# MinhZou/SNGNN

Hardware: NVIDIA B200
Metric: simknn_build_gpairs_per_s (higher is better)
Workload: dtype f16 tensor-core scores + f32 exact rescore

## Files before the change

### sngnn_b200/csrc/sng_simknn.cu

```cuda
#include "sng_common.cuh"
#include <cuda.h>
#include <cuda_fp16.h>
#include <math_constants.h>
#include <stdlib.h>

namespace sng {
namespace knn {

constexpr int BM = 128;
constexpr int BN = 256;
constexpr int BK = 64;
constexpr int kTileBytes = 128 * BK * 2;
constexpr int kUmmaK = 16;
constexpr int kNonEpiThreads = 128;
constexpr int kMaxStages = 10;
constexpr int kMaxD = 4096;
constexpr int kMaxCandTotal = 192;
constexpr uint32_t kPeerMask = 0xFEFFFFFFu;
#ifdef SNG_KNN_INSTRUMENT
constexpr bool kInstr = true;
#else
constexpr bool kInstr = false;
#endif
#ifdef SNG_KNN_EVTRACE
constexpr bool kEvTrace = true;
#else
constexpr bool kEvTrace = false;
#endif
constexpr int kQueue = 256;
constexpr int kSeedGroups = 16;
constexpr float kQScale = 32512.0f, kQOff = 1.0078125f, kQBin = 1.0f / 32512.0f;
__device__ __forceinline__ unsigned short q_of(float v) {
    const int q = __float2int_rd((v + kQOff) * kQScale);
    return (unsigned short)min(max(q, 0), 65535);
}
__device__ __forceinline__ float q_upper(unsigned q) { return ((float)q + 1.5f) * kQBin - kQOff; }

__device__ __forceinline__ uint32_t smem_u32(const void* p) { return (uint32_t)__cvta_generic_to_shared(p); }
__device__ __forceinline__ uint32_t cluster_ctarank() { uint32_t r; asm volatile("mov.u32 %0, %%cluster_ctarank;" : "=r"(r)); return r; }
__device__ __forceinline__ void cluster_sync_all() {
    asm volatile("barrier.cluster.arrive.release.aligned;" ::: "memory");
    asm volatile("barrier.cluster.wait.acquire.aligned;" ::: "memory");
}
__device__ __forceinline__ bool elect_one() {
    uint32_t p;
    asm volatile("{\n\t.reg .pred p;\n\telect.sync _|p, 0xffffffff;\n\tselp.u32 %0, 1, 0, p;\n\t}" : "=r"(p));
    return p != 0;
}
__device__ __forceinline__ void mbar_init(uint32_t bar, uint32_t count) {
    asm volatile("mbarrier.init.shared::cta.b64 [%0], %1;" ::"r"(bar), "r"(count) : "memory");
}
__device__ __forceinline__ void mbar_expect_tx(uint32_t bar, uint32_t bytes) {
    asm volatile("mbarrier.arrive.expect_tx.shared::cta.b64 _, [%0], %1;" ::"r"(bar), "r"(bytes) : "memory");
}
__device__ __forceinline__ void mbar_arrive_cluster(uint32_t bar, uint32_t cta) {
    asm volatile("{\n\t.reg .b32 ra;\n\tmapa.shared::cluster.u32 ra, %0, %1;\n\tmbarrier.arrive.shared::cluster.b64 _, [ra];\n\t}"
                 ::"r"(bar), "r"(cta) : "memory");
}
__device__ __forceinline__ bool mbar_try(uint32_t bar, uint32_t parity) {
    uint32_t done;
    asm volatile("{\n\t.reg .pred p;\n\tmbarrier.try_wait.parity.shared::cta.b64 p, [%1], %2;\n\tselp.u32 %0, 1, 0, p;\n\t}"
                 : "=r"(done) : "r"(bar), "r"(parity) : "memory");
    return done != 0;
}
__device__ __forceinline__ uint32_t mapa_cluster(uint32_t addr, uint32_t cta) {
    uint32_t ra;
    asm volatile("mapa.shared::cluster.u32 %0, %1, %2;" : "=r"(ra) : "r"(addr), "r"(cta));
    return ra;
}
__device__ __forceinline__ void mbar_arrive_remote(uint32_t cluster_addr) {
    asm volatile("mbarrier.arrive.shared::cluster.b64 _, [%0];" ::"r"(cluster_addr) : "memory");
}
__device__ __noinline__ void mbar_wait_slow(uint32_t bar, uint32_t parity) {
    uint32_t done, polls = 0;
    unsigned long long t0 = 0;
    while (true) {
        asm volatile("{\n\t.reg .pred p;\n\tmbarrier.try_wait.parity.shared::cta.b64 p, [%1], %2;\n\tselp.u32 %0, 1, 0, p;\n\t}"
                     : "=r"(done) : "r"(bar), "r"(parity) : "memory");
        if (done) return;
        if (++polls > 4096u) {
            unsigned long long now;
            asm volatile("mov.u64 %0, %%globaltimer;" : "=l"(now));
            if (t0 == 0) t0 = now;
            else if (now - t0 > 4000000000ull) __trap();
        }
    }
}
__device__ __forceinline__ void mbar_wait(uint32_t bar, uint32_t parity) {
    if (!mbar_try(bar, parity)) mbar_wait_slow(bar, parity);
}
__device__ __forceinline__ void tma_load_2d_pair(uint32_t dst, const CUtensorMap* map, uint32_t bar_leader, int c0, int c1) {
    asm volatile("cp.async.bulk.tensor.2d.cta_group::2.shared::cluster.global.mbarrier::complete_tx::bytes [%0], [%1, {%3, %4}], [%2];"
                 ::"r"(dst), "l"(reinterpret_cast<uint64_t>(map)), "r"(bar_leader), "r"(c0), "r"(c1) : "memory");
}
__device__ __forceinline__ void tc_fence_before() { asm volatile("tcgen05.fence::before_thread_sync;" ::: "memory"); }
__device__ __forceinline__ void tc_fence_after() { asm volatile("tcgen05.fence::after_thread_sync;" ::: "memory"); }
__device__ __forceinline__ void umma_f16_pair(uint32_t tmem_d, uint64_t adesc, uint64_t bdesc, uint32_t idesc, uint32_t accumulate) {
    asm volatile("{\n\t.reg .pred p;\n\tsetp.ne.b32 p, %4, 0;\n\ttcgen05.mma.cta_group::2.kind::f16 [%0], %1, %2, %3, p;\n\t}"
                 ::"r"(tmem_d), "l"(adesc), "l"(bdesc), "r"(idesc), "r"(accumulate) : "memory");
}
__device__ __forceinline__ void umma_commit_pair(uint32_t bar) {
    asm volatile("tcgen05.commit.cta_group::2.mbarrier::arrive::one.shared::cluster.multicast::cluster.b64 [%0], %1;"
                 ::"r"(bar), "h"((uint16_t)3) : "memory");
}
__device__ __forceinline__ void tmem_ld32(uint32_t taddr, uint32_t (&v)[32]) {
    asm volatile(
        "tcgen05.ld.sync.aligned.32x32b.x32.b32 "
        "{%0,%1,%2,%3,%4,%5,%6,%7,%8,%9,%10,%11,%12,%13,%14,%15,%16,%17,%18,%19,%20,%21,%22,%23,%24,%25,%26,%27,%28,%29,%30,%31}, [%32];"
        : "=r"(v[0]), "=r"(v[1]), "=r"(v[2]), "=r"(v[3]), "=r"(v[4]), "=r"(v[5]), "=r"(v[6]), "=r"(v[7]), "=r"(v[8]), "=r"(v[9]),
          "=r"(v[10]), "=r"(v[11]), "=r"(v[12]), "=r"(v[13]), "=r"(v[14]), "=r"(v[15]), "=r"(v[16]), "=r"(v[17]), "=r"(v[18]),
          "=r"(v[19]), "=r"(v[20]), "=r"(v[21]), "=r"(v[22]), "=r"(v[23]), "=r"(v[24]), "=r"(v[25]), "=r"(v[26]), "=r"(v[27]),
          "=r"(v[28]), "=r"(v[29]), "=r"(v[30]), "=r"(v[31])
        : "r"(taddr) : "memory");
}
__device__ __forceinline__ void tmem_ld_wait() { asm volatile("tcgen05.wait::ld.sync.aligned;" ::: "memory"); }
__device__ __forceinline__ float max3(float a, float b, float c) {
    float r;
    asm("max.f32 %0, %1, %2, %3;" : "=f"(r) : "f"(a), "f"(b), "f"(c));
    return r;
}
__device__ __forceinline__ float select32(const uint32_t (&v)[32], int i) {
    uint32_t a[16], b[8], c[4], d[2];
#pragma unroll
    for (int j = 0; j < 16; ++j) a[j] = (i & 1) ? v[2 * j + 1] : v[2 * j];
#pragma unroll
    for (int j = 0; j < 8; ++j) b[j] = (i & 2) ? a[2 * j + 1] : a[2 * j];
#pragma unroll
    for (int j = 0; j < 4; ++j) c[j] = (i & 4) ? b[2 * j + 1] : b[2 * j];
#pragma unroll
    for (int j = 0; j < 2; ++j) d[j] = (i & 8) ? c[2 * j + 1] : c[2 * j];
    return __uint_as_float((i & 16) ? d[1] : d[0]);
}

__device__ __forceinline__ uint64_t make_smem_desc(uint32_t saddr) {
    return (uint64_t)((saddr & 0x3FFFFu) >> 4) | ((uint64_t)(1024u >> 4) << 32) | (1ull << 46) | (2ull << 61);
}
constexpr uint32_t kIdesc = (1u << 4) | ((uint32_t)(BN >> 3) << 17) | ((uint32_t)(256 >> 4) << 24);

struct Stage1Params {
    int nq, n, q_offset;
    int kblocks, ksteps_last;
    int stages;
    int stream_a;
    int cand;
    int qcap;
    int nsplit, tiles_total;
    float thr_lo;
    int remove_self;
    int issuers;
    int debug;
    float* cand_val;
    int* cand_idx;
    float* cand_min;
    const float* seeds;
    float* seed_out;
    int seed_q, seed_stride;
    const int* nq_dev;
    const int* row_ids;
    int* phase;
    long long* trace;
};

template <int W, int NI>
__device__ __forceinline__ void issue_split(const Stage1Params& p, uint32_t base, uint32_t a_off, uint32_t b_off, uint32_t bar_full, uint32_t bar_empty,
                                            uint32_t bar_tfull, uint32_t bar_tempty, int t_beg, int t_end, bool issuer, int lane) {
    constexpr uint32_t kIdescHalf = (1u << 4) | ((uint32_t)(128 >> 3) << 17) | ((uint32_t)(256 >> 4) << 24);
    long long* const trc = kInstr ? p.trace : nullptr;
    const uint64_t adesc0 = make_smem_desc(base + a_off);
    const uint64_t bdesc0 = make_smem_desc(base + b_off);
    const int kb2 = p.kblocks == 2;
    const int ks0 = kb2 ? 4 : p.ksteps_last;
    const int ks1 = kb2 ? p.ksteps_last : 0;
    const int nst = p.stages, step = NI * p.kblocks;
    int st0 = (W * p.kblocks) % nst;
    uint32_t ph0 = (uint32_t)((W * p.kblocks) / nst) & 1u;
    for (int tt = W; tt < t_end - t_beg; tt += NI) {
        const int st1 = st0 + 1;
        const uint32_t acc_phase = (uint32_t)(tt >> 1) & 1u;
        const int acc0 = 2 * (tt & 1);
        const uint64_t b0 = bdesc0 + (uint64_t)(st0 * (kTileBytes >> 4)), b1 = bdesc0 + (uint64_t)(st1 * (kTileBytes >> 4));
        mbar_wait(bar_full + 8 * st0, ph0);
        mbar_wait(bar_tempty + 8 * (tt & 1), acc_phase ^ 1);
        tc_fence_after();
#pragma unroll
        for (int h = 0; h < 2; ++h) {
            if (h == 0 && trc && blockIdx.x == 0 && blockIdx.y == 0 && tt < 64 && lane == 0) trc[tt * 8 + 0] = clock64();
            const uint32_t tmem_d = (uint32_t)((acc0 + h) * 128);
            const uint64_t hb = (uint64_t)(h * (kTileBytes >> 5));
            if (issuer) {
#pragma unroll
                for (int ks = 0; ks < 4; ++ks)
                    if (ks < ks0) umma_f16_pair(tmem_d, adesc0 + (uint64_t)(ks * 2), b0 + hb + (uint64_t)(ks * 2), kIdescHalf, ks != 0 ? 1u : 0u);
#pragma unroll
                for (int ks = 0; ks < 4; ++ks)
                    if (ks < ks1) umma_f16_pair(tmem_d, adesc0 + (uint64_t)((kTileBytes >> 4) + ks * 2), b1 + hb + (uint64_t)(ks * 2), kIdescHalf, 1u);
                if (h == 1) umma_commit_pair(bar_empty + 8 * st0);
                umma_commit_pair(bar_tfull + 8 * (acc0 + h));
            }
            __syncwarp();
        }
        if (trc && blockIdx.x == 0 && blockIdx.y == 0 && tt < 64 && lane == 0) trc[tt * 8 + 1] = clock64();
        st0 += step;
        while (st0 >= nst) { st0 -= nst; ph0 ^= 1u; }
    }
}

template <int EW, bool SEED>
__global__ void __cluster_dims__(2, 1, 1) __launch_bounds__(kNonEpiThreads + 128 * EW, 1)
simknn_stage1_kernel(const __grid_constant__ CUtensorMap map_q, const __grid_constant__ CUtensorMap map_db, const Stage1Params p) {
    constexpr int CPT = BN / EW;
    constexpr bool SPLIT = (EW == 4);
    const int dbg = kInstr ? p.debug : 0;
    long long* const trc = kInstr ? p.trace : nullptr;
    const int nq_eff = p.nq_dev ? min(__ldg(p.nq_dev), p.nq) : p.nq;
    if ((int)(blockIdx.x >> 1) * 2 * BM >= nq_eff) return;
    extern __shared__ uint8_t smem_raw[];
    const uint32_t base = (smem_u32(smem_raw) + 1023u) & ~1023u;
    uint8_t* smem = smem_raw + (base - smem_u32(smem_raw));

    const int warp = threadIdx.x >> 5, lane = threadIdx.x & 31;
    const uint32_t rank = cluster_ctarank();
    const uint32_t a_off = 0;
    const uint32_t b_off = a_off + (p.stream_a ? 0u : (uint32_t)p.kblocks * kTileBytes);
    const uint32_t stage_bytes = p.stream_a ? 2u * kTileBytes : (uint32_t)kTileBytes;
    const uint32_t list_off = b_off + (uint32_t)p.stages * stage_bytes;
    const uint32_t thr_off = list_off + (uint32_t)p.cand * BM * 6u;
    const uint32_t q_off = (thr_off + BM * 12u + 15u) & ~15u;
    const uint32_t qcap = (uint32_t)p.qcap;
    const uint32_t bar_off = q_off + qcap * 68u + 16u;
    int* list_idx = reinterpret_cast<int*>(smem + list_off);
    unsigned short* list_val = reinterpret_cast<unsigned short*>(smem + list_off + (size_t)p.cand * BM * 4);
    volatile float* row_thr = reinterpret_cast<volatile float*>(smem + thr_off);
    int* list_cnt = reinterpret_cast<int*>(smem + thr_off + BM * 4);
    int* list_minpos = reinterpret_cast<int*>(smem + thr_off + BM * 8);
    float4* q_ent = reinterpret_cast<float4*>(smem + q_off);
    volatile int* q_flag = reinterpret_cast<volatile int*>(smem + q_off + qcap * 64);
    unsigned* q_head = reinterpret_cast<unsigned*>(smem + q_off + qcap * 68);
    volatile unsigned* q_tail = reinterpret_cast<volatile unsigned*>(smem + q_off + qcap * 68 + 4);
    unsigned* q_done = reinterpret_cast<unsigned*>(smem + q_off + qcap * 68 + 8);
    const uint32_t bar_full = base + bar_off;
    const uint32_t bar_empty = bar_full + 8 * kMaxStages;
    const uint32_t bar_a = bar_empty + 8 * kMaxStages;
    const uint32_t bar_tfull = bar_a + 8;
    const uint32_t bar_tempty = bar_tfull + 32;
    uint32_t* tmem_slot = reinterpret_cast<uint32_t*>(smem + bar_off + 8 * (2 * kMaxStages + 9));

    const int row0 = (int)blockIdx.x * BM;
    const int t_beg = (int)(((long long)p.tiles_total * blockIdx.y) / p.nsplit);
    const int t_end = (int)(((long long)p.tiles_total * (blockIdx.y + 1)) / p.nsplit);
    const int T = t_end - t_beg;
    uint32_t* t0_slot = tmem_slot + 1;

    if (warp == 1 && lane == 0) {
        for (int s = 0; s < p.stages; ++s) { mbar_init(bar_full + 8 * s, 2); mbar_init(bar_empty + 8 * s, 1); }
        mbar_init(bar_a, 2);
        for (int s = 0; s < 4; ++s) { mbar_init(bar_tfull + 8 * s, 1); mbar_init(bar_tempty + 8 * s, SPLIT ? 32 : 2 * 4 * EW); }
        asm volatile("fence.mbarrier_init.release.cluster;" ::: "memory");
    } else if (warp == 2) {
        asm volatile("tcgen05.alloc.cta_group::2.sync.aligned.shared::cta.b32 [%0], 512;" ::"r"(smem_u32(tmem_slot)) : "memory");
        asm volatile("tcgen05.relinquish_alloc_permit.cta_group::2.sync.aligned;" ::: "memory");
    } else if (warp == 3) {
        for (int i = lane; i < BM; i += 32) {
            float tau = p.thr_lo;
            const int grow = row0 + i;
            if (!SEED && grow >= nq_eff) tau = CUDART_INF_F;
            if (!SEED && p.seeds != nullptr && grow < nq_eff) {
                const int srow = p.row_ids ? __ldg(p.row_ids + grow) : grow;
                float g[kSeedGroups];
#pragma unroll
                for (int j = 0; j < kSeedGroups / 4; ++j) {
                    const float4 t4 = __ldg(reinterpret_cast<const float4*>(p.seeds + (size_t)srow * kSeedGroups) + j);
                    g[4 * j] = t4.x; g[4 * j + 1] = t4.y; g[4 * j + 2] = t4.z; g[4 * j + 3] = t4.w;
                }
                const int self = p.q_offset + srow;
                if (p.remove_self && self % p.seed_stride == 0) {
                    const int cs = self / p.seed_stride, sg = ((cs >> 8) & 1) * 8 + ((cs & 255) >> 5);
#pragma unroll
                    for (int j = 0; j < kSeedGroups; ++j) if (j == sg) g[j] = -CUDART_INF_F;
                }
                float cur = CUDART_INF_F;
                for (int r = 0; r < p.seed_q; ++r) {
                    float mx = -CUDART_INF_F;
#pragma unroll
                    for (int j = 0; j < kSeedGroups; ++j) mx = fmaxf(mx, g[j]);
                    bool gone = false;
#pragma unroll
                    for (int j = 0; j < kSeedGroups; ++j) if (!gone && g[j] == mx) { g[j] = -CUDART_INF_F; gone = true; }
                    cur = mx;
                }
                tau = fmaxf(tau, cur);
            }
            row_thr[i] = tau;
            list_cnt[i] = 0;
            list_minpos[i] = 0;
        }
        for (int i = lane; i < (int)qcap; i += 32) q_flag[i] = 0;
        if (lane == 0) { *q_head = 0u; *q_tail = 0u; *q_done = 0u; }
        if (lane == 0 && rank == 0) {
            const uint32_t t0 = (p.phase != nullptr && T > 0) ? (uint32_t)(*reinterpret_cast<volatile int*>(p.phase + blockIdx.y)) % (uint32_t)T : 0u;
            *t0_slot = t0;
        }
    }
    tc_fence_before();
    __syncthreads();
    cluster_sync_all();
    tc_fence_after();
    if (*tmem_slot != 0u) __trap();
    int t_start;
    asm volatile("{\n\t.reg .b32 ra;\n\tmapa.shared::cluster.u32 ra, %1, 0;\n\tld.shared::cluster.u32 %0, [ra];\n\t}"
                 : "=r"(t_start) : "r"(smem_u32(t0_slot)) : "memory");
    t_start += t_beg;

    long long life_clk = 0; unsigned long long life_ns = 0;
    const bool life = trc && threadIdx.x == 0 && blockIdx.y == 0 && (blockIdx.x == 0 || blockIdx.x == gridDim.x - 2);
    if (life) { life_clk = clock64(); asm volatile("mov.u64 %0, %%globaltimer;" : "=l"(life_ns)); }
    if (warp == 0) {
        const bool issuer = elect_one();
        const uint32_t bar_a_leader = bar_a & kPeerMask;
        if (issuer && !p.stream_a) {
            for (int kb = 0; kb < p.kblocks; ++kb)
                tma_load_2d_pair(base + a_off + (uint32_t)kb * kTileBytes, &map_q, bar_a_leader, kb * BK, row0);
            if (rank == 0) mbar_expect_tx(bar_a, 2u * (uint32_t)p.kblocks * kTileBytes);
            else mbar_arrive_cluster(bar_a, 0);
        }
        int stage = 0; uint32_t phase = 0;
        for (int tt = 0, t = t_start; tt < T; ++tt, t = (t + 1 == t_end) ? t_beg : t + 1) {
            if (p.phase != nullptr && rank == 0 && (tt & 63) == 0 && issuer) p.phase[blockIdx.y] = t - t_beg;
            const int brow = t * BN + (int)rank * 128;
            if constexpr (SPLIT) {
                mbar_wait(bar_empty + 8 * stage, phase ^ 1);
                if (issuer) {
                    if (!(dbg & 4)) {
                        for (int kb = 0; kb < p.kblocks; ++kb)
                            tma_load_2d_pair(base + b_off + (uint32_t)(stage + kb) * kTileBytes, &map_db, (bar_full + 8 * stage) & kPeerMask, kb * BK, brow);
                        if (rank == 0) mbar_expect_tx(bar_full + 8 * stage, 2u * (uint32_t)p.kblocks * kTileBytes);
                        else mbar_arrive_cluster(bar_full + 8 * stage, 0);
                    } else {
                        mbar_arrive_cluster(bar_full + 8 * stage, 0);
                    }
                }
                stage += p.kblocks;
                if (stage >= p.stages) { stage = 0; phase ^= 1; }
            } else {
            for (int kb = 0; kb < p.kblocks; ++kb) {
                mbar_wait(bar_empty + 8 * stage, phase ^ 1);
                if (issuer) {
                    if (!(dbg & 4)) {
                        const uint32_t sdst = base + b_off + (uint32_t)stage * stage_bytes;
                        if (p.stream_a) tma_load_2d_pair(sdst, &map_q, (bar_full + 8 * stage) & kPeerMask, kb * BK, row0);
                        tma_load_2d_pair(sdst + (p.stream_a ? (uint32_t)kTileBytes : 0u), &map_db, (bar_full + 8 * stage) & kPeerMask, kb * BK, brow);
                        if (rank == 0) mbar_expect_tx(bar_full + 8 * stage, 2u * stage_bytes);
                        else mbar_arrive_cluster(bar_full + 8 * stage, 0);
                    } else {
                        mbar_arrive_cluster(bar_full + 8 * stage, 0);
                    }
                }
                if (++stage == p.stages) { stage = 0; phase ^= 1; }
            }
            }
        }
    } else if (warp == 1 || warp == 2) {
        const int w = warp - 1;
        if (rank == 0 && w < p.issuers) {
            const bool issuer = elect_one();
            if (!p.stream_a) mbar_wait(bar_a, 0);
            tc_fence_after();
            const uint64_t adesc0 = make_smem_desc(base + a_off);
            const uint64_t bdesc0 = make_smem_desc(base + b_off);
            int stage = 0; uint32_t phase = 0;
            auto advance = [&](int steps) { for (int i = 0; i < steps; ++i) if (++stage == p.stages) { stage = 0; phase ^= 1; } };
            advance(w * p.kblocks);
            if constexpr (SPLIT) {
                if (p.issuers == 1) issue_split<0, 1>(p, base, a_off, b_off, bar_full, bar_empty, bar_tfull, bar_tempty, t_beg, t_end, issuer, lane);
                else if (warp == 1) issue_split<0, 2>(p, base, a_off, b_off, bar_full, bar_empty, bar_tfull, bar_tempty, t_beg, t_end, issuer, lane);
                else issue_split<1, 2>(p, base, a_off, b_off, bar_full, bar_empty, bar_tfull, bar_tempty, t_beg, t_end, issuer, lane);
            } else {
            for (int tt = w; tt < T; tt += p.issuers) {
                const int acc = tt & 1;
                const uint32_t acc_phase = (uint32_t)(tt >> 1) & 1u;
                mbar_wait(bar_tempty + 8 * acc, acc_phase ^ 1);
                tc_fence_after();
                if (trc && blockIdx.x == 0 && blockIdx.y == 0 && tt < 64 && lane == 0) trc[tt * 8 + 0] = clock64();
                const uint32_t tmem_d = (uint32_t)(acc * BN);
                for (int kb = 0; kb < p.kblocks; ++kb) {
                    mbar_wait(bar_full + 8 * stage, phase);
                    tc_fence_after();
                    const int ksteps = (kb == p.kblocks - 1) ? p.ksteps_last : (BK / kUmmaK);
                    const uint64_t adesc = p.stream_a ? bdesc0 + (uint64_t)(stage * 2 * (kTileBytes >> 4)) : adesc0 + (uint64_t)(kb * (kTileBytes >> 4));
                    const uint64_t bdesc = p.stream_a ? adesc + (uint64_t)(kTileBytes >> 4) : bdesc0 + (uint64_t)(stage * (kTileBytes >> 4));
                    if (issuer) {
                        for (int ks = 0; ks < ksteps; ++ks)
                            umma_f16_pair(tmem_d, adesc + (uint64_t)(ks * 2), bdesc + (uint64_t)(ks * 2), kIdesc, (kb | ks) != 0 ? 1u : 0u);
                        umma_commit_pair(bar_empty + 8 * stage);
                        if (kb == p.kblocks - 1) umma_commit_pair(bar_tfull + 8 * acc);
                    }
                    __syncwarp();
                    advance(1);
                }
                if (trc && blockIdx.x == 0 && blockIdx.y == 0 && tt < 64 && lane == 0) trc[tt * 8 + 1] = clock64();
                advance((p.issuers - 1) * p.kblocks);
            }
            }
        }
    } else if (warp == 3) {
        if (!SEED) {
            const int L = p.cand;
            unsigned tail = 0;
            while (true) {
                const unsigned s = (tail + lane) & (qcap - 1);
                const unsigned ready = __ballot_sync(0xffffffffu, q_flag[s] != 0);
                const int nr = ready == 0xffffffffu ? 32 : __ffs(~ready) - 1;
                if (nr == 0) {
                    const unsigned done = *reinterpret_cast<volatile unsigned*>(q_done);
                    const unsigned head = *reinterpret_cast<volatile unsigned*>(q_head);
                    if (done == (unsigned)(4 * EW) && head == tail) break;
                    __nanosleep(200);
                    continue;
                }
                __threadfence_block();
                const bool mine = lane < nr;
                int row = 0, col0 = 0; unsigned mleft = 0u;
                const float* qf = reinterpret_cast<const float*>(q_ent + 4 * s);
                if (mine) {
                    col0 = __float_as_int(qf[11]); row = __float_as_int(qf[12]);
                    const float thr0 = row_thr[row];
#pragma unroll
                    for (int i = 0; i < 11; ++i) mleft |= (qf[i] > thr0 ? 1u : 0u) << i;
                }
                while (__any_sync(0xffffffffu, mleft != 0u)) {
                    const bool has = mleft != 0u;
                    const int i = has ? __ffs(mleft) - 1 : 0;
                    mleft &= mleft - 1u;
                    const float val = has ? qf[i] : 0.f;
                    const int rowk = has ? row : -1 - lane;
                    unsigned pending = __ballot_sync(0xffffffffu, has);
                    while (pending) {
                        const unsigned same = __match_any_sync(0xffffffffu, rowk) & pending;
                        const bool go = has && ((pending >> lane) & 1u) && (__ffs(same) - 1 == lane);
                        if (go) {
                            const float thr = row_thr[row];
                            if (val > thr) {
                                int c = list_cnt[row], slot;
                                if (c < L) { slot = c; list_cnt[row] = ++c; }
                                else slot = list_minpos[row];
                                list_val[slot * BM + row] = q_of(val);
                                list_idx[slot * BM + row] = col0 + 3 * i;
                                if (c == L) {
                                    unsigned mn = list_val[row]; int mp = 0;
#pragma unroll 4
                                    for (int s2 = 1; s2 < L; ++s2) { const unsigned y = list_val[s2 * BM + row]; if (y < mn) { mn = y; mp = s2; } }
                                    list_minpos[row] = mp;
                                    const float tn = q_upper(mn);
                                    if (tn > thr) row_thr[row] = tn;
                                }
                            }
                        }
                        __syncwarp();
                        pending &= ~__ballot_sync(0xffffffffu, go);
                    }
                }
                if (mine) q_flag[s] = 0;
                __threadfence_block();
                __syncwarp();
                tail += (unsigned)nr;
                if (lane == 0) *q_tail = tail;
            }
            __threadfence_block();
            const int lists = p.nsplit;
            for (int i = lane; i < BM * L; i += 32) {
                const int r = i / L, sl = i - r * L, grow = row0 + r;
                if (grow < nq_eff) {
                    const size_t o = ((size_t)grow * lists + blockIdx.y) * L + sl;
                    const bool ok = sl < list_cnt[r];
                    p.cand_val[o] = ok ? q_upper(list_val[sl * BM + r]) : -CUDART_INF_F;
                    p.cand_idx[o] = ok ? list_idx[sl * BM + r] : -1;
                }
            }
            for (int r = lane; r < BM; r += 32) {
                const int grow = row0 + r;
                if (grow < nq_eff) p.cand_min[(size_t)grow * lists + blockIdx.y] = row_thr[r] > p.thr_lo ? row_thr[r] : -CUDART_INF_F;
            }
        }
    } else if (warp >= 4) {
        constexpr int CT = CPT / 32;
        const int quarter = warp & 3, slice = (warp - 4) >> 2;
        const int r = quarter * 32 + lane;
        const int grow = row0 + r;
        const int self_col = p.remove_self ? p.q_offset + ((p.row_ids && grow < nq_eff) ? __ldg(p.row_ids + grow) : grow) : -1;
        const int n = p.n;
        float thr_cur = p.thr_lo;
        long long ev_chunks = 0, ev_n = 0, ev_cyc = 0, ev_max = 0, ev_push = 0;
        float gmax[2 * CT];
#pragma unroll
        for (int i = 0; i < 2 * CT; ++i) gmax[i] = -CUDART_INF_F;

        auto process = [&](uint32_t (&v)[32], int col0, int ci, bool odd) {
            if (dbg & 1) { if (__uint_as_float(v[0] ^ v[31]) == 12345.678f) thr_cur = 0.f; return; }
            float m[11];
            auto tree = [&]() {
#pragma unroll
                for (int i = 0; i < 10; ++i) m[i] = max3(__uint_as_float(v[3 * i]), __uint_as_float(v[3 * i + 1]), __uint_as_float(v[3 * i + 2]));
                m[10] = fmaxf(__uint_as_float(v[30]), __uint_as_float(v[31]));
                const float m0 = max3(m[0], m[1], m[2]), m1 = max3(m[3], m[4], m[5]), m2 = max3(m[6], m[7], m[8]);
                return max3(max3(m0, m1, m2), m[9], m[10]);
            };
            float mx = tree();
            if (SEED) {
                if (col0 + 32 > n) {
                    mx = -CUDART_INF_F;
#pragma unroll
                    for (int i = 0; i < 32; ++i) if (col0 + i < n) mx = fmaxf(mx, __uint_as_float(v[i]));
                }
                gmax[ci] = fmaxf(gmax[ci], odd ? -CUDART_INF_F : mx);
                gmax[CT + ci] = fmaxf(gmax[CT + ci], odd ? mx : -CUDART_INF_F);
                return;
            }
            const bool cnt_on = kEvTrace && trc && blockIdx.x == 0 && blockIdx.y == 0 && threadIdx.x == kNonEpiThreads;
            if (cnt_on) ++ev_chunks;
            if (__any_sync(0xffffffffu, mx > thr_cur)) {
                const long long ev0 = cnt_on ? clock64() : 0;
                if (dbg & 8) return;
                if ((unsigned)(self_col - col0) < 32u || col0 + 32 > n) {
#pragma unroll
                    for (int i = 0; i < 32; ++i) if (col0 + i == self_col || col0 + i >= n) v[i] = 0xff800000u;
                    mx = tree();
                }
                if (mx > thr_cur) {
                    const unsigned at = atomicAdd(q_head, 1u);
                    while ((int)(at - *q_tail) >= (int)qcap) __nanosleep(20);
                    const unsigned s = at & (qcap - 1);
                    q_ent[4 * s] = make_float4(m[0], m[1], m[2], m[3]);
                    q_ent[4 * s + 1] = make_float4(m[4], m[5], m[6], m[7]);
                    q_ent[4 * s + 2] = make_float4(m[8], m[9], m[10], __int_as_float(col0));
                    q_ent[4 * s + 3] = make_float4(__int_as_float(r), 0.f, 0.f, 0.f);
                    __threadfence_block();
                    q_flag[s] = 1;
                    if (cnt_on) ++ev_push;
                }
                __syncwarp();
                thr_cur = fmaxf(thr_cur, row_thr[r]);
                if (cnt_on) {
                    const long long dt = clock64() - ev0;
                    ++ev_n; ev_cyc += dt; ev_max = dt > ev_max ? dt : ev_max;
                }
            }
        };

        uint32_t va[32], vb[32];
        const int tile_col = SPLIT ? 128 * (slice >> 1) + 64 * (slice & 1) : slice * CPT;
        uint32_t taddr_e = ((uint32_t)(quarter * 32) << 16) + (uint32_t)(SPLIT ? (slice & 1) * 128 + (slice >> 1) * 64 : slice * CPT);
        uint32_t bar_tf_e = bar_tfull + 8u * (SPLIT ? (uint32_t)(slice & 1) : 0u);
        uint32_t bar_te_e = mapa_cluster(bar_tempty, 0);
        for (int tt = 0, t = t_start; tt < T; ++tt, t = (t + 1 == t_end) ? t_beg : t + 1) {
            asm volatile("" : "+r"(taddr_e), "+r"(bar_tf_e), "+r"(bar_te_e));
            const uint32_t par = (uint32_t)tt & 1u;
            const uint32_t acc_phase = (uint32_t)(tt >> 1) & 1u;
            mbar_wait(bar_tf_e + par * (SPLIT ? 16u : 8u), acc_phase);
            tc_fence_after();
            const bool tr = trc && blockIdx.x == 0 && blockIdx.y == 0 && tt < 64 && threadIdx.x == kNonEpiThreads;
            if (tr) trc[tt * 8 + 2] = clock64();
            if (!SEED) thr_cur = fmaxf(thr_cur, row_thr[r]);
            const uint32_t taddr = taddr_e + par * (uint32_t)(SPLIT ? 256 : BN);
            const int col0 = t * BN + tile_col;
            const bool odd = (t & 1) != 0;
            if (CPT == 64) {
                if (!(dbg & 2)) {
                    tmem_ld32(taddr, va);
                    tmem_ld32(taddr + 32, vb);
                    tmem_ld_wait();
                }
                tc_fence_before();
                __syncwarp();
                if (lane == 0) mbar_arrive_remote(bar_te_e + 8u * par);
                if (tr) trc[tt * 8 + 3] = clock64();
                process(va, col0, 0, odd);
                process(vb, col0 + 32, CT > 1 ? 1 : 0, odd);
            } else {
                tmem_ld32(taddr, va);
#pragma unroll
                for (int c = 0; c < CT; c += 2) {
                    tmem_ld_wait();
                    tmem_ld32(taddr + (c + 1) * 32, vb);
                    process(va, col0 + c * 32, c, odd);
                    tmem_ld_wait();
                    if (c + 2 < CT) tmem_ld32(taddr + (c + 2) * 32, va);
                    else {
                        tc_fence_before();
                        __syncwarp();
                        if (lane == 0) mbar_arrive_remote(bar_te_e + 8u * par);
                    }
                    process(vb, col0 + (c + 1) * 32, c + 1, odd);
                }
            }
        }
        if (SEED) {
            if (grow < nq_eff) {
#pragma unroll
                for (int i = 0; i < 2 * CT; ++i)
                    p.seed_out[(size_t)grow * kSeedGroups + (i / CT) * 8 + (tile_col >> 5) + (i % CT)] = gmax[i];
            }
        } else {
            __syncwarp();
            __threadfence_block();
            if (lane == 0) atomicAdd(q_done, 1u);
            if (kEvTrace && trc && blockIdx.x == 0 && blockIdx.y == 0 && threadIdx.x == kNonEpiThreads) {
                trc[525] = ev_chunks; trc[520] = ev_n; trc[521] = ev_push; trc[526] = ev_cyc; trc[527] = ev_max;
            }
        }
    }
    tc_fence_before();
    __syncthreads();
    if (life) {
        unsigned long long ns1; asm volatile("mov.u64 %0, %%globaltimer;" : "=l"(ns1));
        long long* o = trc + 512 + (blockIdx.x == 0 ? 0 : 4);
        o[0] = clock64() - life_clk; o[1] = (long long)(ns1 - life_ns); o[2] = T; o[3] = blockIdx.x;
    }
    cluster_sync_all();
    if (warp == 2) {
        tc_fence_after();
        asm volatile("tcgen05.dealloc.cta_group::2.sync.aligned.b32 %0, 512;" ::"r"(0u) : "memory");
    }
}

__device__ __forceinline__ float dot_seq(const float* __restrict__ a, const float* __restrict__ b, int d4) {
    float s = 0.f;
    for (int k = 0; k < d4; ++k) {
        const float4 x = ldg4(a + 4 * k), y = ldg4(b + 4 * k);
        s = fmaf(x.x, y.x, s); s = fmaf(x.y, y.y, s); s = fmaf(x.z, y.z, s); s = fmaf(x.w, y.w, s);
    }
    return s;
}
__device__ __forceinline__ bool better(float sa, int ia, float sb, int ib) { return sa > sb || (sa == sb && ia < ib); }

__global__ void __launch_bounds__(256) simknn_rescore_kernel(
    const float* __restrict__ xq, const float* __restrict__ xall, int64_t ld32, int d4, int nq, int n, int q_offset, int remove_self, int m_total,
    int nsplit, int top_k, float thr, float eps, const float* __restrict__ cand_val, const int* __restrict__ cand_idx,
    const float* __restrict__ cand_min,
    int* __restrict__ idx_out, float* __restrict__ sim_out, int* __restrict__ cnt_out, int* __restrict__ fb_rows, int* __restrict__ n_fallback,
    const int* __restrict__ nq_dev, const int* __restrict__ row_map) {
    extern __shared__ float sm2[];
    const int warp = threadIdx.x >> 5, lane = threadIdx.x & 31;
    const int m3 = 3 * m_total;
    float* sc = sm2 + (size_t)warp * 2 * m3;
    int* id = reinterpret_cast<int*>(sc + m3);
    if (nq_dev) nq = min(nq, __ldg(nq_dev));
    for (int f = blockIdx.x * 8 + warp; f < nq; f += gridDim.x * 8) {
        const int row = row_map ? __ldg(row_map + f) : f;
        const float* a = xq + (int64_t)row * ld32;
        const int self_col = remove_self ? q_offset + row : -1;
        {
            bool nz = false;
            for (int k4 = lane; k4 < d4; k4 += 32) { const float4 v = ldg4(a + 4 * k4); nz = nz || v.x != 0.f || v.y != 0.f || v.z != 0.f || v.w != 0.f; }
            if (!__any_sync(0xffffffffu, nz)) {
                const int avail = n - ((self_col >= 0 && self_col < n) ? 1 : 0);
                const int cnt0 = 0.0f >= thr ? min(top_k, avail) : 0;
                for (int t = lane; t < top_k; t += 32) {
                    const int j = (self_col >= 0 && t >= self_col) ? t + 1 : t;
                    idx_out[(size_t)row * top_k + t] = t < cnt0 ? j : -1;
                    sim_out[(size_t)row * top_k + t] = 0.f;
                }
                if (lane == 0) cnt_out[row] = cnt0;
                __syncwarp();
                continue;
            }
        }
        for (int m = lane; m < m_total; m += 32)
            sc[m] = __ldg(cand_idx + (size_t)f * m_total + m) >= 0 ? __ldg(cand_val + (size_t)f * m_total + m) : -CUDART_INF_F;
        __syncwarp();
        float tk = CUDART_INF_F; int ntrip = 0;
        for (int m0 = 0; m0 < m_total; m0 += 32) {
            const int m = m0 + lane;
            const float v = m < m_total ? sc[m] : -CUDART_INF_F;
            int above = 0;
            for (int o = 0; o < m_total; ++o) above += sc[o] > v ? 1 : 0;
            if (v > -CUDART_INF_F && above < top_k) tk = fminf(tk, v);
            ntrip += __popc(__ballot_sync(0xffffffffu, v > -CUDART_INF_F));
        }
#pragma unroll
        for (int o = 16; o > 0; o >>= 1) tk = fminf(tk, __shfl_xor_sync(0xffffffffu, tk, o));
        const float cutoff = ntrip >= top_k ? tk - 2.0f * eps - 2.0f * kQBin : -CUDART_INF_F;
        __syncwarp();
        int nvalid = 0;
        for (int m0 = 0; m0 < m3; m0 += 32) {
            const int m = m0 + lane;
            int j = -1; float s = -CUDART_INF_F;
            if (m < m3) {
                const int base = __ldg(cand_idx + (size_t)f * m_total + m / 3), e = m % 3;
                if (base >= 0 && __ldg(cand_val + (size_t)f * m_total + m / 3) >= cutoff && (e < 2 || (base & 31) != 30) && base + e < n &&
                    base + e != self_col) {
                    j = base + e;
                    s = dot_seq(a, xall + (int64_t)j * ld32, d4);
                }
                sc[m] = s; id[m] = j;
            }
            nvalid += __popc(__ballot_sync(0xffffffffu, j >= 0 && s >= thr));
        }
        __syncwarp();
        const int cnt = min(nvalid, top_k);
        float kth = thr;
        for (int m0 = 0; m0 < m3; m0 += 32) {
            const int m = m0 + lane;
            int rank = 0x7fffffff; float s = 0.f; int j = -1;
            if (m < m3) {
                s = sc[m]; j = id[m];
                if (j >= 0 && s >= thr) {
                    rank = 0;
                    for (int o = 0; o < m3; ++o) rank += (id[o] >= 0 && better(sc[o], id[o], s, j)) ? 1 : 0;
                }
            }
            if (rank < top_k) {
                idx_out[(size_t)row * top_k + rank] = j;
                sim_out[(size_t)row * top_k + rank] = s;
            }
            const unsigned hit = __ballot_sync(0xffffffffu, rank == top_k - 1);
            if (hit) kth = __shfl_sync(0xffffffffu, s, __ffs(hit) - 1);
        }
        for (int t = cnt + lane; t < top_k; t += 32) { idx_out[(size_t)row * top_k + t] = -1; sim_out[(size_t)row * top_k + t] = 0.f; }
        float bound = -CUDART_INF_F;
        for (int s0 = lane; s0 < nsplit; s0 += 32) bound = fmaxf(bound, __ldg(cand_min + (size_t)f * nsplit + s0) + eps);
#pragma unroll
        for (int o = 16; o > 0; o >>= 1) bound = fmaxf(bound, __shfl_xor_sync(0xffffffffu, bound, o));
        if (lane == 0) {
            cnt_out[row] = cnt;
            if (!(kth > bound)) fb_rows[atomicAdd(n_fallback, 1)] = row;
        }
        __syncwarp();
    }
}

constexpr int kRetryRowsMin = 16384, kRetryRowsMax = 262144;
static int retry_rows(int64_t nq) {
    int64_t c = (nq + 255) / 256 * 256;
    if (c < kRetryRowsMin) c = kRetryRowsMin;
    if (c > kRetryRowsMax) c = kRetryRowsMax;
    return (int)c;
}
constexpr int kRetryRounds = 48;
__global__ void __launch_bounds__(256) simknn_retry_rounds_kernel(const int* __restrict__ fb_rows, const int* __restrict__ n_fb, int cap, int rounds,
                                                                 int* __restrict__ round_cnt, int* __restrict__ fb2_rows, int* __restrict__ n_fb2) {
    const int nfb = *n_fb;
    for (int r = threadIdx.x; r < rounds; r += blockDim.x) round_cnt[r] = max(0, min(cap, nfb - r * cap));
    for (long long f = (long long)rounds * cap + threadIdx.x; f < nfb; f += blockDim.x) fb2_rows[atomicAdd(n_fb2, 1)] = fb_rows[f];
}
__global__ void __launch_bounds__(256) simknn_retry_gather_kernel(const uint16_t* __restrict__ xq, int64_t ldb, const int* __restrict__ fb_rows,
                                                                 const int* __restrict__ n_round, uint16_t* __restrict__ xq_retry) {
    const int nr = *n_round;
    const int lane = threadIdx.x & 31;
    const int w = blockIdx.x * 8 + (threadIdx.x >> 5), nw = gridDim.x * 8;
    const int64_t vec = ldb / 8;
    for (int f = w; f < nr; f += nw) {
        const uint4* src = reinterpret_cast<const uint4*>(xq + (int64_t)fb_rows[f] * ldb);
        uint4* dst = reinterpret_cast<uint4*>(xq_retry + (int64_t)f * ldb);
        for (int64_t i = lane; i < vec; i += 32) dst[i] = src[i];
    }
}

constexpr int kChunk = 8192;
constexpr int kFbWaveRows = 4096;
constexpr int kFbWaves = 4;

struct Pick { float s; int i; };
__device__ __forceinline__ Pick block_argmax(float bs, int bi, float* red_s, int* red_i) {
#pragma unroll
    for (int o = 16; o > 0; o >>= 1) {
        const float os = __shfl_xor_sync(0xffffffffu, bs, o);
        const int oi = __shfl_xor_sync(0xffffffffu, bi, o);
        if (better(os, oi, bs, bi)) { bs = os; bi = oi; }
    }
    if ((threadIdx.x & 31) == 0) { red_s[threadIdx.x >> 5] = bs; red_i[threadIdx.x >> 5] = bi; }
    __syncthreads();
    bs = red_s[0]; bi = red_i[0];
    for (int w = 1; w < (int)(blockDim.x >> 5); ++w) if (better(red_s[w], red_i[w], bs, bi)) { bs = red_s[w]; bi = red_i[w]; }
    __syncthreads();
    return Pick{bs, bi};
}

__global__ void __launch_bounds__(256) simknn_fb_scan_kernel(
    const float* __restrict__ xq, const float* __restrict__ xall, int64_t ld32, int d4, int n, int q_offset, int top_k, float thr,
    int remove_self, const int* __restrict__ fb_rows, const int* __restrict__ n_fallback, int wave, int n_chunks,
    float* __restrict__ part_s, int* __restrict__ part_i) {
    __shared__ float sc[kChunk];
    __shared__ float red_s[8];
    __shared__ int red_i[8];
    const int f_lo = wave * kFbWaveRows;
    const int f_hi = min(*n_fallback, f_lo + kFbWaveRows);
    const long long items = (long long)max(f_hi - f_lo, 0) * n_chunks;
    for (long long it = blockIdx.x; it < items; it += gridDim.x) {
        const int fl = (int)(it / n_chunks), ch = (int)(it % n_chunks);
        const int row = fb_rows[f_lo + fl];
        const float* a = xq + (int64_t)row * ld32;
        const int self_col = remove_self ? q_offset + row : -1;
        const int c0 = ch * kChunk, cn = min(kChunk, n - c0);
        for (int j = threadIdx.x; j < cn; j += blockDim.x)
            sc[j] = (c0 + j == self_col) ? -CUDART_INF_F : dot_seq(a, xall + (int64_t)(c0 + j) * ld32, d4);
        __syncthreads();
        float prev_s = CUDART_INF_F; int prev_i = -1;
        const size_t o = ((size_t)fl * n_chunks + ch) * top_k;
        for (int t = 0; t < top_k; ++t) {
            float bs = -CUDART_INF_F; int bi = 0x7fffffff;
            for (int j = threadIdx.x; j < cn; j += blockDim.x) {
                const float s = sc[j];
                const int gi = c0 + j;
                const bool after = s < prev_s || (s == prev_s && gi > prev_i);
                if (after && s >= thr && better(s, gi, bs, bi)) { bs = s; bi = gi; }
            }
            const Pick pk = block_argmax(bs, bi, red_s, red_i);
            prev_s = pk.s; prev_i = pk.i;
            if (threadIdx.x == 0) { part_s[o + t] = pk.s; part_i[o + t] = pk.i == 0x7fffffff ? -1 : pk.i; }
            if (pk.i == 0x7fffffff) {
                for (int u = t + 1 + threadIdx.x; u < top_k; u += blockDim.x) { part_s[o + u] = -CUDART_INF_F; part_i[o + u] = -1; }
                break;
            }
        }
        __syncthreads();
    }
}

__global__ void __launch_bounds__(256) simknn_fb_merge_kernel(
    const int* __restrict__ fb_rows, const int* __restrict__ n_fallback, int wave, int n_chunks, int top_k,
    const float* __restrict__ part_s, const int* __restrict__ part_i, int* __restrict__ idx_out, float* __restrict__ sim_out,
    int* __restrict__ cnt_out) {
    __shared__ float red_s[8];
    __shared__ int red_i[8];
    const int f_lo = wave * kFbWaveRows;
    const int f_hi = min(*n_fallback, f_lo + kFbWaveRows);
    const int m = n_chunks * top_k;
    for (int fl = blockIdx.x; fl < f_hi - f_lo; fl += gridDim.x) {
        const int row = fb_rows[f_lo + fl];
        const float* ps = part_s + (size_t)fl * m;
        const int* pi = part_i + (size_t)fl * m;
        float prev_s = CUDART_INF_F; int prev_i = -1; int cnt = 0;
        for (int t = 0; t < top_k; ++t) {
            float bs = -CUDART_INF_F; int bi = 0x7fffffff;
            for (int j = threadIdx.x; j < m; j += blockDim.x) {
                const int gi = pi[j];
                if (gi < 0) continue;
                const float s = ps[j];
                const bool after = s < prev_s || (s == prev_s && gi > prev_i);
                if (after && better(s, gi, bs, bi)) { bs = s; bi = gi; }
            }
            const Pick pk = block_argmax(bs, bi, red_s, red_i);
            if (pk.i == 0x7fffffff) break;
            prev_s = pk.s; prev_i = pk.i;
            if (threadIdx.x == 0) { idx_out[(size_t)row * top_k + t] = pk.i; sim_out[(size_t)row * top_k + t] = pk.s; }
            ++cnt;
        }
        if (threadIdx.x == 0) {
            for (int t = cnt; t < top_k; ++t) { idx_out[(size_t)row * top_k + t] = -1; sim_out[(size_t)row * top_k + t] = 0.f; }
            cnt_out[row] = cnt;
        }
        __syncthreads();
    }
}

__global__ void __launch_bounds__(256) simknn_fb_stream_kernel(
    const float* __restrict__ xq, const float* __restrict__ xall, int64_t ld32, int d4, int n, int q_offset, int top_k, float thr,
    int remove_self, const int* __restrict__ fb_rows, const int* __restrict__ n_fallback, int f_start,
    int* __restrict__ idx_out, float* __restrict__ sim_out, int* __restrict__ cnt_out) {
    __shared__ float sc[kChunk];
    __shared__ float red_s[8];
    __shared__ int red_i[8];
    __shared__ float best_s[SNG_KNN_MAX_TOPK];
    __shared__ int best_i[SNG_KNN_MAX_TOPK];
    __shared__ int best_n;
    const int nfb = *n_fallback;
    for (int f = f_start + blockIdx.x; f < nfb; f += gridDim.x) {
        const int row = fb_rows[f];
        const float* a = xq + (int64_t)row * ld32;
        const int self_col = remove_self ? q_offset + row : -1;
        if (threadIdx.x == 0) best_n = 0;
        __syncthreads();
        for (int c0 = 0; c0 < n; c0 += kChunk) {
            const int cn = min(kChunk, n - c0);
            for (int j = threadIdx.x; j < cn; j += blockDim.x)
                sc[j] = (c0 + j == self_col) ? -CUDART_INF_F : dot_seq(a, xall + (int64_t)(c0 + j) * ld32, d4);
            __syncthreads();
            float prev_s = CUDART_INF_F; int prev_i = -1;
            for (int t = 0; t < top_k; ++t) {
                const int bn = best_n;
                const float kth = bn == top_k ? best_s[top_k - 1] : -CUDART_INF_F;
                float bs = -CUDART_INF_F; int bi = 0x7fffffff;
                for (int j = threadIdx.x; j < cn; j += blockDim.x) {
                    const float sv = sc[j];
                    const int gi = c0 + j;
                    const bool after = sv < prev_s || (sv == prev_s && gi > prev_i);
                    if (after && sv >= thr && sv > kth && better(sv, gi, bs, bi)) { bs = sv; bi = gi; }
                }
                const Pick pk = block_argmax(bs, bi, red_s, red_i);
                if (pk.i == 0x7fffffff) break;
                prev_s = pk.s; prev_i = pk.i;
                if (threadIdx.x == 0) {
                    int pos = bn < top_k ? bn : top_k - 1;
                    while (pos > 0 && best_s[pos - 1] < pk.s) { best_s[pos] = best_s[pos - 1]; best_i[pos] = best_i[pos - 1]; --pos; }
                    best_s[pos] = pk.s; best_i[pos] = pk.i;
                    if (bn < top_k) best_n = bn + 1;
                }
                __syncthreads();
            }
            __syncthreads();
        }
        if (threadIdx.x == 0) {
            const int bn = best_n;
            for (int t = 0; t < top_k; ++t) {
                idx_out[(size_t)row * top_k + t] = t < bn ? best_i[t] : -1;
                sim_out[(size_t)row * top_k + t] = t < bn ? best_s[t] : 0.f;
            }
            cnt_out[row] = bn;
        }
        __syncthreads();
    }
}

typedef CUresult (*EncodeTiledFn)(CUtensorMap*, CUtensorMapDataType, cuuint32_t, void*, const cuuint64_t*, const cuuint64_t*,
                                  const cuuint32_t*, const cuuint32_t*, CUtensorMapInterleave, CUtensorMapSwizzle,
                                  CUtensorMapL2promotion, CUtensorMapFloatOOBfill);

static EncodeTiledFn get_encode_fn() {
    static EncodeTiledFn fn = nullptr;
    if (!fn) {
        void* p = nullptr;
        cudaDriverEntryPointQueryResult q;
        if (cudaGetDriverEntryPoint("cuTensorMapEncodeTiled", &p, cudaEnableDefault, &q) == cudaSuccess && q == cudaDriverEntryPointSuccess)
            fn = reinterpret_cast<EncodeTiledFn>(p);
        else
            cudaGetLastError();
    }
    return fn;
}

static int make_map(CUtensorMap* map, const uint16_t* ptr, int64_t rows, int64_t ld, int64_t row_stride = 1) {
    EncodeTiledFn enc = get_encode_fn();
    if (!enc) { set_error("cuTensorMapEncodeTiled is not available from the driver"); return SNG_ERR_CUDA; }
    cuuint64_t gdim[2] = {(cuuint64_t)ld, (cuuint64_t)rows};
    cuuint64_t gstr[1] = {(cuuint64_t)ld * 2 * (cuuint64_t)row_stride};
    cuuint32_t box[2] = {(cuuint32_t)BK, (cuuint32_t)BM};
    cuuint32_t estr[2] = {1, 1};
    CUresult r = enc(map, CU_TENSOR_MAP_DATA_TYPE_FLOAT16, 2, const_cast<uint16_t*>(ptr), gdim, gstr, box, estr,
                     CU_TENSOR_MAP_INTERLEAVE_NONE, CU_TENSOR_MAP_SWIZZLE_128B, CU_TENSOR_MAP_L2_PROMOTION_L2_256B,
                     CU_TENSOR_MAP_FLOAT_OOB_FILL_NONE);
    if (r != CUDA_SUCCESS) { set_error("cuTensorMapEncodeTiled failed with CUresult %d (rows=%lld ld=%lld)", (int)r, (long long)rows, (long long)ld); return SNG_ERR_CUDA; }
    return SNG_OK;
}

struct Plan {
    int ew, stages, cand, qcap, nsplit, kblocks, ksteps_last, tiles, stream_a;
    int seed_stride, seed_q;
    size_t smem;
    int lists() const { return nsplit; }
};

static int seed_quantile(int top_k, int stride, double tol) {
    const double pr = 1.0 / stride;
    double pmf = 1.0;
    for (int i = 0; i < top_k; ++i) pmf *= 1.0 - pr;
    double tail = 1.0 - pmf;
    for (int q = 1; q <= top_k; ++q) {
        if (tail <= tol) return q;
        pmf *= (double)(top_k - q + 1) / q * pr / (1.0 - pr);
        tail -= pmf;
    }
    return top_k + 1;
}

static size_t smem_bytes(int ew, int kblocks, int stages, int cand, int qcap, bool stream_a = false) {
    (void)ew;
    return 1024 + (stream_a ? (size_t)stages * 2 * kTileBytes : (size_t)kblocks * kTileBytes + (size_t)stages * kTileBytes) + (size_t)cand * BM * 6 + BM * 12 +
           16 + (size_t)qcap * 68 + 16 + 8 * (2 * kMaxStages + 9) + 16;
}

static int g_debug_env = 0;
static int env_int(const char* name, int lo, int hi) {
    if (!g_debug_env) return 0;
    const char* e = getenv(name);
    if (!e) return 0;
    const int v = atoi(e);
    return (v >= lo && v <= hi) ? v : 0;
}
static bool env_flag(const char* name) { return g_debug_env && getenv(name) != nullptr; }
}
int debug_env_int(const char* name, int lo, int hi) { return knn::env_int(name, lo, hi); }
namespace knn {

static int cand_for(int top_k, int margin) {
    const int o = env_int("SNG_KNN_CAND", top_k, 128);
    if (o) return o;
    return (top_k + margin + 1) / 2 * 2;
}

static int make_plan(Plan* pl, int64_t nq, int64_t n, int64_t d, int top_k, int cand, int force_ew) {
    const size_t kMaxSmem = 227 * 1024;
    if (!force_ew) force_ew = env_int("SNG_KNN_EW", 1, 4) == 3 ? 0 : env_int("SNG_KNN_EW", 1, 4);
    const int d16 = (int)((d + 15) / 16 * 16);
    pl->kblocks = (d16 + BK - 1) / BK;
    pl->ksteps_last = (d16 - (pl->kblocks - 1) * BK) / kUmmaK;
    pl->tiles = (int)((n + BN - 1) / BN);
    pl->ew = 0;
    pl->stream_a = 0;
    const int ew_pref = d16 <= 128 ? 4 : (d16 <= 320 ? 2 : 1);
    if (force_ew == 4 && pl->kblocks > 2) force_ew = 2;
    static const int kMargins[] = {22, 14, 8, 4};
    for (int pass = 0; pass < 2 && !pl->ew; ++pass) {
        for (int ew = force_ew ? force_ew : ew_pref; ew >= 1 && !pl->ew; ew >>= 1) {
            for (int mi = 0; mi < (top_k > 0 ? (pass ? 4 : 2) : 1) && !pl->ew; ++mi) {
                const int c = top_k > 0 ? cand_for(top_k, kMargins[mi]) : cand;
                if (c > kMaxCandTotal) continue;
                for (int qc = kQueue; qc >= 64 && !pl->ew; qc /= 4) {
                    int want = pl->kblocks * 4 < kMaxStages ? (pl->kblocks * 4 > 4 ? pl->kblocks * 4 : 4) : kMaxStages;
                    if (env_int("SNG_KNN_STAGES", 2, kMaxStages)) want = env_int("SNG_KNN_STAGES", 2, kMaxStages);
                    for (int st = want; st >= (pass ? 2 : 3); --st) {
                        if (ew == 4 && st % pl->kblocks != 0) continue;
                        const size_t sz = smem_bytes(ew, pl->kblocks, st, c, qc);
                        if (sz <= kMaxSmem) { pl->ew = ew; pl->stages = st; pl->smem = sz; pl->cand = c; pl->qcap = qc; break; }
                    }
                }
            }
            if (force_ew) break;
        }
    }
    if (!pl->ew && force_ew != 4) {
        static const int kMarginsS[] = {22, 14, 8, 4};
        for (int mi = 0; mi < (top_k > 0 ? 4 : 1) && !pl->ew; ++mi) {
            const int c = top_k > 0 ? cand_for(top_k, kMarginsS[mi]) : cand;
            if (c > kMaxCandTotal) continue;
            for (int qc = kQueue; qc >= 64 && !pl->ew; qc /= 4)
                for (int st = 5; st >= 2; --st) {
                    const size_t sz = smem_bytes(1, pl->kblocks, st, c, qc, true);
                    if (sz <= kMaxSmem) { pl->ew = 1; pl->stages = st; pl->smem = sz; pl->cand = c; pl->qcap = qc; pl->stream_a = 1; break; }
                }
        }
    }
    if (!pl->ew) { set_error("simknn: d=%lld top_k=%d does not fit in shared memory", (long long)d, top_k); return SNG_ERR_UNSUPPORTED; }
    if (pl->smem <= kMaxSmem / 2) pl->smem = kMaxSmem / 2 + 1024;
    const int sms = sm_count() > 0 ? sm_count() : 148;
    const int64_t ctas = 2 * ((nq + 2 * BM - 1) / (2 * BM));
    int ns = (int)((3ll * sms + ctas - 1) / ctas);
    if (ns > 8) ns = 8;
    if (ns > pl->tiles) ns = pl->tiles;
    while (ns > 1 && ns * pl->cand > kMaxCandTotal) --ns;
    if (ns < 1) ns = 1;
    pl->nsplit = ns;
    pl->seed_stride = pl->seed_q = 0;
    const bool forced = env_int("SNG_KNN_SEED_S", 2, 256) != 0;
    if (top_k > 0 && !env_flag("SNG_KNN_NOSEED")) {
        if (forced) {
            const int stride = env_int("SNG_KNN_SEED_S", 2, 256);
            int q = env_int("SNG_KNN_SEED_Q", 1, kSeedGroups - 2);
            if (!q) q = seed_quantile(top_k, stride, 2e-5);
            if (pl->tiles / stride >= 8 && q <= kSeedGroups - 4) { pl->seed_stride = stride; pl->seed_q = q; }
        } else {
            for (int stride = pl->tiles >= 2048 ? 32 : (pl->tiles >= 512 ? 16 : (pl->tiles / 32 > 4 ? pl->tiles / 32 : 4)); stride <= 64 && !pl->seed_stride; stride *= 2) {
                const int q = seed_quantile(top_k, stride, 2e-5);
                if (pl->tiles / stride >= 8 && q <= kSeedGroups - 4) { pl->seed_stride = stride; pl->seed_q = q; }
            }
        }
    }
    return SNG_OK;
}

template <int EW, bool SEED>
static cudaError_t launch_ew(dim3 grid, size_t smem, cudaStream_t st, const CUtensorMap& mq, const CUtensorMap& mdb, const Stage1Params& p) {
    cudaError_t e = cudaFuncSetAttribute(simknn_stage1_kernel<EW, SEED>, cudaFuncAttributeMaxDynamicSharedMemorySize, (int)smem);
    if (e != cudaSuccess) return e;
    simknn_stage1_kernel<EW, SEED><<<grid, kNonEpiThreads + 128 * EW, smem, st>>>(mq, mdb, p);
    return cudaSuccess;
}

static int launch_stage1(const Plan& pl, const uint16_t* xq, const uint16_t* xall, int64_t ldb, int64_t nq, int64_t q_offset, int64_t n,
                         float thr_lo, int remove_self, float* cand_val, int* cand_idx, float* cand_min, const float* seeds,
                         float* seed_out, int* phase, cudaStream_t st, const int* nq_dev = nullptr, const int* row_ids = nullptr) {
    const bool seed_pass = seed_out != nullptr;
    const int64_t n_db = seed_pass ? (n + pl.seed_stride - 1) / pl.seed_stride : n;
    CUtensorMap mq, mdb;
    if (int rc = make_map(&mq, xq, nq, ldb)) return rc;
    if (int rc = make_map(&mdb, xall, n_db, ldb, seed_pass ? pl.seed_stride : 1)) return rc;
    Stage1Params p;
    p.nq = (int)nq; p.n = (int)n_db; p.q_offset = (int)q_offset;
    p.kblocks = pl.kblocks; p.ksteps_last = pl.ksteps_last; p.stages = pl.stages; p.stream_a = pl.stream_a; p.cand = seed_pass ? 0 : pl.cand; p.qcap = pl.qcap;
    p.nsplit = seed_pass ? 1 : pl.nsplit; p.tiles_total = (int)((n_db + BN - 1) / BN); p.thr_lo = thr_lo; p.remove_self = remove_self;
    p.debug = env_int("SNG_KNN_DEBUG", 1, 63);
    p.issuers = env_int("SNG_KNN_ISSUERS", 1, 2) ? env_int("SNG_KNN_ISSUERS", 1, 2) : (pl.kblocks <= 3 ? 2 : 1);
    if (pl.stream_a) p.issuers = 1;
    p.cand_val = cand_val; p.cand_idx = cand_idx; p.cand_min = cand_min;
    p.phase = seed_pass ? nullptr : phase;
    p.nq_dev = nq_dev; p.row_ids = row_ids;
    p.seeds = seed_pass ? nullptr : seeds; p.seed_out = seed_out; p.seed_q = pl.seed_q; p.seed_stride = pl.seed_stride > 0 ? pl.seed_stride : 1;
    dim3 grid((unsigned)(2 * ((nq + 2 * BM - 1) / (2 * BM))), (unsigned)p.nsplit);
    p.trace = nullptr;
    if (env_flag("SNG_KNN_TRACE") && !seed_pass) {
        cudaMalloc(&p.trace, (64 * 8 + 16) * sizeof(long long));
        cudaMemset(p.trace, 0, (64 * 8 + 16) * sizeof(long long));
    }
    cudaError_t e;
    if (seed_pass) e = pl.ew == 4 ? launch_ew<4, true>(grid, pl.smem, st, mq, mdb, p)
                     : pl.ew == 2 ? launch_ew<2, true>(grid, pl.smem, st, mq, mdb, p)
                                  : launch_ew<1, true>(grid, pl.smem, st, mq, mdb, p);
    else e = pl.ew == 4 ? launch_ew<4, false>(grid, pl.smem, st, mq, mdb, p)
           : pl.ew == 2 ? launch_ew<2, false>(grid, pl.smem, st, mq, mdb, p)
                        : launch_ew<1, false>(grid, pl.smem, st, mq, mdb, p);
    if (e != cudaSuccess) { cudaGetLastError(); set_error("simknn stage 1: cudaFuncSetAttribute(%zu B smem): %s", pl.smem, cudaGetErrorString(e)); return SNG_ERR_CUDA; }
    if (p.trace) {
        long long h[64 * 8 + 16];
        cudaStreamSynchronize(st);
        cudaMemcpy(h, p.trace, sizeof(h), cudaMemcpyDeviceToHost);
        cudaFree(p.trace);
        fprintf(stderr, "tile  mma:tempty_ok  [4]  [5]  [6]  mma:issued  epi:tfull_ok  epi:released   (cycles since tile 0's tempty_ok; split mode: [4] = half 0 issued, [5] = half 1 stage free)\n");
        for (int t = 0; t < 64; ++t)
            fprintf(stderr, "%4d %10lld %10lld %10lld %10lld %10lld %10lld %10lld\n", t, h[8 * t] - h[0], h[8 * t + 4] - h[0], h[8 * t + 5] - h[0],
                    h[8 * t + 6] - h[0], h[8 * t + 1] - h[0], h[8 * t + 2] - h[0], h[8 * t + 3] - h[0]);
        fprintf(stderr, "CTA 0 warp 4: %lld warp-chunks, %lld slow-path events, %lld pushes (%lld %lld %lld); "
                "event cycles: mean %.0f max %lld\n", h[525], h[520], h[521], h[522], h[523], h[524], (double)h[526] / (double)(h[520] > 0 ? h[520] : 1), h[527]);
        for (int c = 0; c < 2; ++c) {
            const long long* o = h + 512 + 4 * c;
            if (o[1] > 0) fprintf(stderr, "CTA %lld lifetime: %lld cycles, %lld ns -> %.0f MHz, %lld tiles, %.0f cycles/tile\n", o[3], o[0], o[1],
                                  1e3 * (double)o[0] / (double)o[1], o[2], (double)o[0] / (double)(o[2] > 0 ? o[2] : 1));
        }
    }
    return check_launch(seed_pass ? "simknn seed pass" : "simknn stage 1");
}

static int check_common(const char* fn, const void* xq, const void* xall, int64_t ldb, int64_t nq, int64_t q_offset, int64_t n, int64_t d) {
    if (!xq || !xall) { set_error("%s: null operand", fn); return SNG_ERR_ARG; }
    if (nq <= 0 || n <= 0 || d <= 0 || q_offset < 0 || n >= (1ll << 31) || nq >= (1ll << 31)) { set_error("%s: bad nq/n/d/q_offset", fn); return SNG_ERR_ARG; }
    if (ldb % 8 != 0 || ldb < (d + 15) / 16 * 16) { set_error("%s: ldb=%lld must be a multiple of 8 and >= d rounded up to 16", fn, (long long)ldb); return SNG_ERR_ARG; }
    if (((uintptr_t)xq | (uintptr_t)xall) & 15) { set_error("%s: FP16 operands must be 16-byte aligned", fn); return SNG_ERR_ARG; }
    if (d > kMaxD) { set_error("%s: d=%lld > %d not supported", fn, (long long)d, kMaxD); return SNG_ERR_UNSUPPORTED; }
    return SNG_OK;
}

constexpr float kScoreEps = 0.0009765625f + 1.2e-4f;
static float score_eps(int64_t d) { return 0.0009765625f + 1.2e-4f * (d > 640 ? (float)d / 640.0f : 1.0f); }
static int64_t retry_ld(int64_t d) { return (d + 15) / 16 * 16 + 64; }

}
}

using namespace sng;
using namespace sng::knn;

static size_t align256(size_t x) { return (x + 255) / 256 * 256; }

extern "C" int sng_set_debug_env(int enabled) { const int was = sng::knn::g_debug_env; sng::knn::g_debug_env = enabled ? 1 : 0; return was; }

extern "C" size_t sng_simknn_workspace_bytes(int64_t nq, int64_t n, int64_t d, int top_k) {
    if (nq <= 0 || n <= 0 || d <= 0 || top_k <= 0 || top_k > SNG_KNN_MAX_TOPK) return 0;
    Plan pl;
    if (make_plan(&pl, nq, n, d, top_k, 0, 0)) return 0;
    const size_t slots = (size_t)nq * pl.lists() * pl.cand;
    const size_t part = (size_t)kFbWaveRows * ((n + kChunk - 1) / kChunk) * top_k;
    return align256(slots * 4) * 2 + align256((size_t)nq * pl.lists() * 4) + align256((size_t)nq * 4) + 2 * align256(part * 4) +
           align256((size_t)nq * kSeedGroups * 4) + 256 +
           align256((size_t)retry_rows(nq) * retry_ld(d) * 2) + 2 * align256((size_t)retry_rows(nq) * kMaxCandTotal * 4) + align256((size_t)retry_rows(nq) * 8 * 4) +
           align256((size_t)nq * 4) + 256 + 1024;
}

extern "C" int sng_simknn_plan(int64_t nq, int64_t n, int64_t d, int top_k, int32_t* out8) {
    SNG_REQUIRE(out8 && nq > 0 && n > 0 && d > 0 && top_k >= 1 && top_k <= SNG_KNN_MAX_TOPK, "sng_simknn_plan: bad arguments");
    Plan pl;
    if (int rc = make_plan(&pl, nq, n, d, top_k, 0, 0)) return rc;
    out8[0] = pl.ew; out8[1] = pl.cand; out8[2] = pl.nsplit; out8[3] = pl.seed_stride; out8[4] = pl.seed_q; out8[5] = pl.stages;
    out8[6] = pl.kblocks; out8[7] = pl.lists();
    return SNG_OK;
}

extern "C" int sng_simknn_seed(const uint16_t* xq, const uint16_t* xall, int64_t ldb, int64_t nq, int64_t n, int64_t d, int seed_stride,
                               int force_ew, float* seeds_out, void* stream) {
    if (int rc = check_common("sng_simknn_seed", xq, xall, ldb, nq, 0, n, d)) return rc;
    SNG_REQUIRE(seeds_out && seed_stride >= 1 && seed_stride <= 256, "sng_simknn_seed: bad seed_stride / output");
    SNG_REQUIRE(force_ew == 0 || force_ew == 1 || force_ew == 2 || force_ew == 4, "sng_simknn_seed: force_ew must be 0, 1, 2 or 4");
    Plan pl;
    if (int rc = make_plan(&pl, nq, n, d, 0, 8, force_ew)) return rc;
    pl.seed_stride = seed_stride; pl.seed_q = 1;
    return launch_stage1(pl, xq, xall, ldb, nq, 0, n, -3.0e38f, 0, nullptr, nullptr, nullptr, nullptr, seeds_out, nullptr, (cudaStream_t)stream);
}

extern "C" int sng_simknn_stage1(const uint16_t* xq, const uint16_t* xall, int64_t ldb, int64_t nq, int64_t q_offset, int64_t n, int64_t d,
                                 int cand, float thr_lo, int remove_self, int32_t* cand_idx, float* cand_val, float* cand_min,
                                 int force_ew, int force_nsplit, int* lists_out, const float* seeds, int seed_q, int seed_stride,
                                 int32_t* sweep_phase, void* stream) {
    if (int rc = check_common("sng_simknn_stage1", xq, xall, ldb, nq, q_offset, n, d)) return rc;
    SNG_REQUIRE(cand >= 8 && cand <= 128 && cand_idx && cand_val && cand_min, "sng_simknn_stage1: bad cand / outputs");
    SNG_REQUIRE(force_ew == 0 || force_ew == 1 || force_ew == 2 || force_ew == 4, "sng_simknn_stage1: force_ew must be 0, 1, 2 or 4");
    Plan pl;
    if (int rc = make_plan(&pl, nq, n, d, 0, cand, force_ew)) return rc;
    if (force_nsplit > 0) pl.nsplit = force_nsplit < pl.tiles ? force_nsplit : pl.tiles;
    SNG_REQUIRE(pl.lists() * cand <= kMaxCandTotal, "sng_simknn_stage1: nsplit*ew*cand = %d exceeds %d", pl.lists() * cand, kMaxCandTotal);
    if (lists_out) *lists_out = pl.lists();
    SNG_REQUIRE(!seeds || (seed_q >= 1 && seed_q <= kSeedGroups - 2 && seed_stride >= 1),
                "sng_simknn_stage1: seeds need 1 <= seed_q <= %d, seed_stride >= 1", kSeedGroups - 2);
    pl.seed_q = seeds ? seed_q : 0; pl.seed_stride = seeds ? seed_stride : 0;
    return launch_stage1(pl, xq, xall, ldb, nq, q_offset, n, thr_lo, remove_self, cand_val, cand_idx, cand_min, seeds, nullptr, sweep_phase, (cudaStream_t)stream);
}

extern "C" int sng_simknn_build(const uint16_t* xq, const uint16_t* xall, int64_t ldb, const float* xq32, const float* xall32, int64_t ld32,
                                int64_t nq, int64_t q_offset, int64_t n, int64_t d, int top_k, float thr, int remove_self,
                                int32_t* idx, float* sim, int32_t* cnt, int32_t* n_fallback, int32_t* n_retry, void* workspace,
                                size_t workspace_bytes, void* stream) {
    if (int rc = check_common("sng_simknn_build", xq, xall, ldb, nq, q_offset, n, d)) return rc;
    SNG_REQUIRE(xq32 && xall32 && ld32 % 4 == 0 && ld32 >= d, "sng_simknn_build: FP32 rows must be padded to a multiple of 4 floats (ld32=%lld)", (long long)ld32);
    SNG_REQUIRE(top_k >= 1 && top_k <= SNG_KNN_MAX_TOPK, "sng_simknn_build: top_k=%d out of [1,%d]", top_k, SNG_KNN_MAX_TOPK);
    SNG_REQUIRE(idx && sim && cnt && n_fallback && workspace, "sng_simknn_build: null output / workspace");
    SNG_REQUIRE(ldb <= retry_ld(d), "sng_simknn_build: ldb=%lld > %lld (rows padded far beyond d)", (long long)ldb, (long long)retry_ld(d));
    const float eps = score_eps(d);
    if (workspace_bytes < sng_simknn_workspace_bytes(nq, n, d, top_k)) { set_error("sng_simknn_build: workspace too small (%zu < %zu)", workspace_bytes, sng_simknn_workspace_bytes(nq, n, d, top_k)); return SNG_ERR_WORKSPACE; }
    Plan pl;
    if (int rc = make_plan(&pl, nq, n, d, top_k, 0, 0)) return rc;
    cudaStream_t st = (cudaStream_t)stream;
    const int m_total = pl.lists() * pl.cand;
    uint8_t* w = reinterpret_cast<uint8_t*>(((uintptr_t)workspace + 255) & ~(uintptr_t)255);
    float* cand_val = reinterpret_cast<float*>(w); w += align256((size_t)nq * m_total * 4);
    int* cand_idx = reinterpret_cast<int*>(w); w += align256((size_t)nq * m_total * 4);
    float* cand_min = reinterpret_cast<float*>(w); w += align256((size_t)nq * pl.lists() * 4);
    int* fb_rows = reinterpret_cast<int*>(w); w += align256((size_t)nq * 4);
    const int n_chunks = (int)((n + kChunk - 1) / kChunk);
    const size_t part = (size_t)kFbWaveRows * n_chunks * top_k;
    float* part_s = reinterpret_cast<float*>(w); w += align256(part * 4);
    int* part_i = reinterpret_cast<int*>(w); w += align256(part * 4);
    float* seeds = reinterpret_cast<float*>(w); w += align256((size_t)nq * kSeedGroups * 4);
    int* phase = reinterpret_cast<int*>(w); w += 256;
    const int kRetryRows = retry_rows(nq);
    uint16_t* xq_retry = reinterpret_cast<uint16_t*>(w); w += align256((size_t)kRetryRows * retry_ld(d) * 2);
    float* rcand_val = reinterpret_cast<float*>(w); w += align256((size_t)kRetryRows * kMaxCandTotal * 4);
    int* rcand_idx = reinterpret_cast<int*>(w); w += align256((size_t)kRetryRows * kMaxCandTotal * 4);
    float* rcand_min = reinterpret_cast<float*>(w); w += align256((size_t)kRetryRows * 8 * 4);
    int* fb2_rows = reinterpret_cast<int*>(w); w += align256((size_t)nq * 4);
    int* n_fb1 = reinterpret_cast<int*>(w);
    Plan pr;
    bool retry = false;
    if (!env_flag("SNG_KNN_NORETRY")) {
        const int want = top_k + 32 <= 64 ? 64 : (top_k + 32 <= 96 ? 96 : 128);
        for (int rcand = want; rcand >= top_k + 8 && !retry; rcand -= 16) {
            if (make_plan(&pr, kRetryRows, n, d, 0, rcand, pl.ew) != SNG_OK || pr.ew != pl.ew) continue;
            pr.seed_stride = pr.seed_q = 0;
            pr.nsplit = kMaxCandTotal / rcand < pr.tiles ? kMaxCandTotal / rcand : pr.tiles;
            if (pr.nsplit < 1) pr.nsplit = 1;
            if (pr.tiles >= 64) {
                const int rc8 = ((top_k + 14 > kMaxCandTotal / 8 ? top_k + 14 : kMaxCandTotal / 8) + 1) / 2 * 2;
                Plan p8;
                if (rc8 < rcand && 8 * rc8 <= kMaxCandTotal && make_plan(&p8, kRetryRows, n, d, 0, rc8, pl.ew) == SNG_OK && p8.ew == pl.ew) {
                    pr = p8; pr.seed_stride = pr.seed_q = 0; pr.nsplit = 8;
                }
            }
            retry = true;
        }
    }
    if (cudaMemsetAsync(phase, 0, 8 * sizeof(int), st) != cudaSuccess) return check_launch("sng_simknn_build memset");
    if (cudaMemsetAsync(n_fb1, 0, sizeof(int), st) != cudaSuccess) return check_launch("sng_simknn_build memset");
    if (cudaMemsetAsync(n_fallback, 0, sizeof(int), st) != cudaSuccess) return check_launch("sng_simknn_build memset");
    const float thr_lo = thr - 1.01f * eps;
    if (pl.seed_stride > 0)
        if (int rc = launch_stage1(pl, xq, xall, ldb, nq, q_offset, n, thr_lo, remove_self, nullptr, nullptr, nullptr, nullptr, seeds, nullptr, st)) return rc;
    if (int rc = launch_stage1(pl, xq, xall, ldb, nq, q_offset, n, thr_lo, remove_self, cand_val, cand_idx, cand_min,
                               pl.seed_stride > 0 ? seeds : nullptr, nullptr, env_flag("SNG_KNN_NOPHASE") ? nullptr : phase, st)) return rc;
    const int d4 = (int)((d + 3) / 4);
    int* flag_rows = retry ? fb_rows : fb2_rows;
    int* flag_cnt = retry ? n_fb1 : n_fallback;
    {
        const int blocks = (int)((nq + 7) / 8 < (int64_t)sm_count() * 8 ? (nq + 7) / 8 : (int64_t)sm_count() * 8);
        simknn_rescore_kernel<<<blocks > 0 ? blocks : 1, 256, (size_t)8 * 2 * 3 * m_total * 4, st>>>(
            xq32, xall32, ld32, d4, (int)nq, (int)n, (int)q_offset, remove_self, m_total, pl.lists(), top_k, thr, eps, cand_val, cand_idx, cand_min,
            idx, sim, cnt, flag_rows, flag_cnt, nullptr, nullptr);
        if (int rc = check_launch("simknn stage 2")) return rc;
    }
    if (retry) {
        if (pl.seed_stride > 0) { pr.seed_stride = pl.seed_stride; pr.seed_q = pl.seed_q + 4 < kSeedGroups - 4 ? pl.seed_q + 4 : kSeedGroups - 4; }
        cudaStreamCaptureStatus cap_status = cudaStreamCaptureStatusNone;
        if (cudaStreamIsCapturing(st, &cap_status) != cudaSuccess) { cudaGetLastError(); cap_status = cudaStreamCaptureStatusNone; }
        const bool capturing = cap_status != cudaStreamCaptureStatusNone;
        int flagged = 0, rounds = 1, cap = kRetryRows;
        if (capturing) {
            cap = kRetryRowsMin < kRetryRows ? kRetryRowsMin : kRetryRows;
        } else {
            if (cudaMemcpyAsync(&flagged, n_fb1, sizeof(int), cudaMemcpyDeviceToHost, st) != cudaSuccess || cudaStreamSynchronize(st) != cudaSuccess)
                return check_launch("sng_simknn_build flagged-row count");
            rounds = (flagged + cap - 1) / cap;
            if (rounds > kRetryRounds) rounds = kRetryRounds;
        }
        int* round_cnt = phase + 16;
        if (rounds > 0) simknn_retry_rounds_kernel<<<1, 256, 0, st>>>(fb_rows, n_fb1, cap, rounds, round_cnt, fb2_rows, n_fallback);
        const int mr = pr.lists() * pr.cand;
        for (int r = 0; r < rounds; ++r) {
            const int* rows_r = fb_rows + (size_t)r * cap;
            const int n_r = capturing ? cap : (flagged - r * cap < cap ? flagged - r * cap : cap);
            const int n_launch = (n_r + 2 * BM - 1) / (2 * BM) * (2 * BM);
            simknn_retry_gather_kernel<<<(sm_count() > 0 ? sm_count() : 148) * 2, 256, 0, st>>>(xq, ldb, rows_r, round_cnt + r, xq_retry);
            if (int rc = launch_stage1(pr, xq_retry, xall, ldb, n_launch, q_offset, n, thr_lo, remove_self, rcand_val, rcand_idx, rcand_min,
                                       pl.seed_stride > 0 ? seeds : nullptr, nullptr, nullptr, st, round_cnt + r, rows_r)) return rc;
            const int rblocks = (n_launch + 7) / 8 < 4096 ? (n_launch + 7) / 8 : 4096;
            simknn_rescore_kernel<<<rblocks, 256, (size_t)8 * 2 * 3 * mr * 4, st>>>(
                xq32, xall32, ld32, d4, n_launch, (int)n, (int)q_offset, remove_self, mr, pr.lists(), top_k, thr, eps, rcand_val, rcand_idx, rcand_min,
                idx, sim, cnt, fb2_rows, n_fallback, round_cnt + r, rows_r);
        }
        if (int rc = check_launch("simknn retry pass")) return rc;
    }
    if (n_retry) {
        if (cudaMemcpyAsync(n_retry, retry ? n_fb1 : n_fallback, sizeof(int), cudaMemcpyDeviceToDevice, st) != cudaSuccess)
            return check_launch("sng_simknn_build n_retry");
    }
    const int fb_grid = (sm_count() > 0 ? sm_count() : 148) * 4;
    for (int wave = 0; wave < kFbWaves; ++wave) {
        simknn_fb_scan_kernel<<<fb_grid, 256, 0, st>>>(xq32, xall32, ld32, d4, (int)n, (int)q_offset, top_k, thr, remove_self, fb2_rows, n_fallback,
                                                      wave, n_chunks, part_s, part_i);
        simknn_fb_merge_kernel<<<fb_grid, 256, 0, st>>>(fb2_rows, n_fallback, wave, n_chunks, top_k, part_s, part_i, idx, sim, cnt);
    }
    simknn_fb_stream_kernel<<<fb_grid, 256, 0, st>>>(xq32, xall32, ld32, d4, (int)n, (int)q_offset, top_k, thr, remove_self, fb2_rows,
                                                    n_fallback, kFbWaves * kFbWaveRows, idx, sim, cnt);
    return check_launch("simknn stage 3");
}
```

Baseline: 6822.

## Exploit symmetry in self-kNN build to compute only half the similarity tiles

When queries equal the database (self-join, single split), each CTA pair now sweeps only about half of the column tiles, a circular window ending at its diagonal tile. Off-diagonal scores are also pushed as candidates to the transposed row through per-column global lists, gated by per-column thresholds that are published from row thresholds. The rescore kernel merges these column lists and uses an overflow max as an extra bound. The goal is to roughly halve the tensor-core GEMM work, at the cost of global atomics, extra queue traffic, threshold staleness that may trigger more fallbacks, and additional workspace memory.

```diff
diff --git a/sngnn_b200/csrc/sng_simknn.cu b/sngnn_b200/csrc/sng_simknn.cu
--- a/sngnn_b200/csrc/sng_simknn.cu
+++ b/sngnn_b200/csrc/sng_simknn.cu
@@ -35,6 +35,8 @@
     return (unsigned short)min(max(q, 0), 65535);
 }
 __device__ __forceinline__ float q_upper(unsigned q) { return ((float)q + 1.5f) * kQBin - kQOff; }
+__device__ __forceinline__ int fkey(float f) { const int b = __float_as_int(f); return b ^ ((b >> 31) & 0x7fffffff); }
+__device__ __forceinline__ float fkey_inv(int k) { return __int_as_float(k ^ ((k >> 31) & 0x7fffffff)); }
 
 __device__ __forceinline__ uint32_t smem_u32(const void* p) { return (uint32_t)__cvta_generic_to_shared(p); }
 __device__ __forceinline__ uint32_t cluster_ctarank() { uint32_t r; asm volatile("mov.u32 %0, %%cluster_ctarank;" : "=r"(r)); return r; }
@@ -159,11 +161,45 @@
     const int* row_ids;
     int* phase;
     long long* trace;
+    int sym;
+    int col_cap;
+    float* col_thr;
+    int* col_cnt;
+    int* col_ovf;
+    int* col_idx;
+    unsigned short* col_val;
 };
+
+__device__ __forceinline__ float seed_threshold(const float* seeds, int srow, int self, int remove_self, int seed_stride, int seed_q, float thr_lo) {
+    float tau = thr_lo;
+    if (seeds == nullptr) return tau;
+    float g[kSeedGroups];
+#pragma unroll
+    for (int j = 0; j < kSeedGroups / 4; ++j) {
+        const float4 t4 = __ldg(reinterpret_cast<const float4*>(seeds + (size_t)srow * kSeedGroups) + j);
+        g[4 * j] = t4.x; g[4 * j + 1] = t4.y; g[4 * j + 2] = t4.z; g[4 * j + 3] = t4.w;
+    }
+    if (remove_self && self % seed_stride == 0) {
+        const int cs = self / seed_stride, sg = ((cs >> 8) & 1) * 8 + ((cs & 255) >> 5);
+#pragma unroll
+        for (int j = 0; j < kSeedGroups; ++j) if (j == sg) g[j] = -CUDART_INF_F;
+    }
+    float cur = CUDART_INF_F;
+    for (int r = 0; r < seed_q; ++r) {
+        float mx = -CUDART_INF_F;
+#pragma unroll
+        for (int j = 0; j < kSeedGroups; ++j) mx = fmaxf(mx, g[j]);
+        bool gone = false;
+#pragma unroll
+        for (int j = 0; j < kSeedGroups; ++j) if (!gone && g[j] == mx) { g[j] = -CUDART_INF_F; gone = true; }
+        cur = mx;
+    }
+    return fmaxf(tau, cur);
+}
 
 template <int W, int NI>
 __device__ __forceinline__ void issue_split(const Stage1Params& p, uint32_t base, uint32_t a_off, uint32_t b_off, uint32_t bar_full, uint32_t bar_empty,
-                                            uint32_t bar_tfull, uint32_t bar_tempty, int t_beg, int t_end, bool issuer, int lane) {
+                                            uint32_t bar_tfull, uint32_t bar_tempty, int T, bool issuer, int lane) {
     constexpr uint32_t kIdescHalf = (1u << 4) | ((uint32_t)(128 >> 3) << 17) | ((uint32_t)(256 >> 4) << 24);
     long long* const trc = kInstr ? p.trace : nullptr;
     const uint64_t adesc0 = make_smem_desc(base + a_off);
@@ -174,7 +210,7 @@
     const int nst = p.stages, step = NI * p.kblocks;
     int st0 = (W * p.kblocks) % nst;
     uint32_t ph0 = (uint32_t)((W * p.kblocks) / nst) & 1u;
-    for (int tt = W; tt < t_end - t_beg; tt += NI) {
+    for (int tt = W; tt < T; tt += NI) {
         const int st1 = st0 + 1;
         const uint32_t acc_phase = (uint32_t)(tt >> 1) & 1u;
         const int acc0 = 2 * (tt & 1);
@@ -248,8 +284,20 @@
     const int row0 = (int)blockIdx.x * BM;
     const int t_beg = (int)(((long long)p.tiles_total * blockIdx.y) / p.nsplit);
     const int t_end = (int)(((long long)p.tiles_total * (blockIdx.y + 1)) / p.nsplit);
-    const int T = t_end - t_beg;
+    const int pair = (int)(blockIdx.x >> 1);
+    struct Sweep { int beg, len, last; };
+    auto sweep = [&]() {
+        Sweep w{t_beg, t_end - t_beg, t_end - 1};
+        if (p.sym) {
+            const int Tt = p.tiles_total;
+            w.len = (Tt - 1) / 2 + 1 + ((Tt % 2 == 0 && pair >= Tt / 2) ? 1 : 0);
+            w.beg = pair - (w.len - 1) + (pair < w.len - 1 ? Tt : 0);
+            w.last = pair;
+        }
+        return w;
+    };
     uint32_t* t0_slot = tmem_slot + 1;
+    auto next_tile = [&](int t, const Sweep& w) { return t == w.last ? w.beg : (t + 1 == p.tiles_total ? 0 : t + 1); };
 
     if (warp == 1 && lane == 0) {
         for (int s = 0; s < p.stages; ++s) { mbar_init(bar_full + 8 * s, 2); mbar_init(bar_empty + 8 * s, 1); }
@@ -264,31 +312,9 @@
             float tau = p.thr_lo;
             const int grow = row0 + i;
             if (!SEED && grow >= nq_eff) tau = CUDART_INF_F;
-            if (!SEED && p.seeds != nullptr && grow < nq_eff) {
+            if (!SEED && grow < nq_eff) {
                 const int srow = p.row_ids ? __ldg(p.row_ids + grow) : grow;
-                float g[kSeedGroups];
-#pragma unroll
-                for (int j = 0; j < kSeedGroups / 4; ++j) {
-                    const float4 t4 = __ldg(reinterpret_cast<const float4*>(p.seeds + (size_t)srow * kSeedGroups) + j);
-                    g[4 * j] = t4.x; g[4 * j + 1] = t4.y; g[4 * j + 2] = t4.z; g[4 * j + 3] = t4.w;
-                }
-                const int self = p.q_offset + srow;
-                if (p.remove_self && self % p.seed_stride == 0) {
-                    const int cs = self / p.seed_stride, sg = ((cs >> 8) & 1) * 8 + ((cs & 255) >> 5);
-#pragma unroll
-                    for (int j = 0; j < kSeedGroups; ++j) if (j == sg) g[j] = -CUDART_INF_F;
-                }
-                float cur = CUDART_INF_F;
-                for (int r = 0; r < p.seed_q; ++r) {
-                    float mx = -CUDART_INF_F;
-#pragma unroll
-                    for (int j = 0; j < kSeedGroups; ++j) mx = fmaxf(mx, g[j]);
-                    bool gone = false;
-#pragma unroll
-                    for (int j = 0; j < kSeedGroups; ++j) if (!gone && g[j] == mx) { g[j] = -CUDART_INF_F; gone = true; }
-                    cur = mx;
-                }
-                tau = fmaxf(tau, cur);
+                tau = seed_threshold(p.seeds, srow, p.q_offset + srow, p.remove_self, p.seed_stride, p.seed_q, p.thr_lo);
             }
             row_thr[i] = tau;
             list_cnt[i] = 0;
@@ -297,8 +323,14 @@
         for (int i = lane; i < (int)qcap; i += 32) q_flag[i] = 0;
         if (lane == 0) { *q_head = 0u; *q_tail = 0u; *q_done = 0u; }
         if (lane == 0 && rank == 0) {
-            const uint32_t t0 = (p.phase != nullptr && T > 0) ? (uint32_t)(*reinterpret_cast<volatile int*>(p.phase + blockIdx.y)) % (uint32_t)T : 0u;
-            *t0_slot = t0;
+            const Sweep sw = sweep();
+            int o = 0;
+            if (p.phase != nullptr && sw.len > 0) {
+                const int ph = t_beg + (int)((uint32_t)(*reinterpret_cast<volatile int*>(p.phase + blockIdx.y)) % (uint32_t)(t_end - t_beg));
+                o = (ph - sw.beg + p.tiles_total) % p.tiles_total;
+                if (o >= sw.len) o = 0;
+            }
+            *t0_slot = (uint32_t)((sw.beg + o) % p.tiles_total);
         }
     }
     tc_fence_before();
@@ -309,7 +341,6 @@
     int t_start;
     asm volatile("{\n\t.reg .b32 ra;\n\tmapa.shared::cluster.u32 ra, %1, 0;\n\tld.shared::cluster.u32 %0, [ra];\n\t}"
                  : "=r"(t_start) : "r"(smem_u32(t0_slot)) : "memory");
-    t_start += t_beg;
 
     long long life_clk = 0; unsigned long long life_ns = 0;
     const bool life = trc && threadIdx.x == 0 && blockIdx.y == 0 && (blockIdx.x == 0 || blockIdx.x == gridDim.x - 2);
@@ -324,7 +355,8 @@
             else mbar_arrive_cluster(bar_a, 0);
         }
         int stage = 0; uint32_t phase = 0;
-        for (int tt = 0, t = t_start; tt < T; ++tt, t = (t + 1 == t_end) ? t_beg : t + 1) {
+        const Sweep sw = sweep();
+        for (int tt = 0, t = t_start; tt < sw.len; ++tt, t = next_tile(t, sw)) {
             if (p.phase != nullptr && rank == 0 && (tt & 63) == 0 && issuer) p.phase[blockIdx.y] = t - t_beg;
             const int brow = t * BN + (int)rank * 128;
             if constexpr (SPLIT) {
@@ -363,6 +395,7 @@
         const int w = warp - 1;
         if (rank == 0 && w < p.issuers) {
             const bool issuer = elect_one();
+            const int T = sweep().len;
             if (!p.stream_a) mbar_wait(bar_a, 0);
             tc_fence_after();
             const uint64_t adesc0 = make_smem_desc(base + a_off);
@@ -371,9 +404,9 @@
             auto advance = [&](int steps) { for (int i = 0; i < steps; ++i) if (++stage == p.stages) { stage = 0; phase ^= 1; } };
             advance(w * p.kblocks);
             if constexpr (SPLIT) {
-                if (p.issuers == 1) issue_split<0, 1>(p, base, a_off, b_off, bar_full, bar_empty, bar_tfull, bar_tempty, t_beg, t_end, issuer, lane);
-                else if (warp == 1) issue_split<0, 2>(p, base, a_off, b_off, bar_full, bar_empty, bar_tfull, bar_tempty, t_beg, t_end, issuer, lane);
-                else issue_split<1, 2>(p, base, a_off, b_off, bar_full, bar_empty, bar_tfull, bar_tempty, t_beg, t_end, issuer, lane);
+                if (p.issuers == 1) issue_split<0, 1>(p, base, a_off, b_off, bar_full, bar_empty, bar_tfull, bar_tempty, T, issuer, lane);
+                else if (warp == 1) issue_split<0, 2>(p, base, a_off, b_off, bar_full, bar_empty, bar_tfull, bar_tempty, T, issuer, lane);
+                else issue_split<1, 2>(p, base, a_off, b_off, bar_full, bar_empty, bar_tfull, bar_tempty, T, issuer, lane);
             } else {
             for (int tt = w; tt < T; tt += p.issuers) {
                 const int acc = tt & 1;
@@ -423,9 +456,19 @@
                 const float* qf = reinterpret_cast<const float*>(q_ent + 4 * s);
                 if (mine) {
                     col0 = __float_as_int(qf[11]); row = __float_as_int(qf[12]);
-                    const float thr0 = row_thr[row];
-#pragma unroll
-                    for (int i = 0; i < 11; ++i) mleft |= (qf[i] > thr0 ? 1u : 0u) << i;
+                    if (row >= 0) {
+                        const float thr0 = row_thr[row];
+#pragma unroll
+                        for (int i = 0; i < 11; ++i) mleft |= (qf[i] > thr0 ? 1u : 0u) << i;
+                    } else {
+                        const int slot = atomicAdd(p.col_cnt + col0, 1);
+                        if (slot < p.col_cap) {
+                            p.col_idx[(size_t)col0 * p.col_cap + slot] = __float_as_int(qf[1]);
+                            p.col_val[(size_t)col0 * p.col_cap + slot] = q_of(qf[0]);
+                        } else {
+                            atomicMax(p.col_ovf + col0, fkey(qf[0]));
+                        }
+                    }
                 }
                 while (__any_sync(0xffffffffu, mleft != 0u)) {
                     const bool has = mleft != 0u;
@@ -451,7 +494,10 @@
                                     for (int s2 = 1; s2 < L; ++s2) { const unsigned y = list_val[s2 * BM + row]; if (y < mn) { mn = y; mp = s2; } }
                                     list_minpos[row] = mp;
                                     const float tn = q_upper(mn);
-                                    if (tn > thr) row_thr[row] = tn;
+                                    if (tn > thr) {
+                                        row_thr[row] = tn;
+                                        if (p.sym && row0 + row < p.n) p.col_thr[row0 + row] = tn;
+                                    }
                                 }
                             }
                         }
@@ -494,7 +540,7 @@
 #pragma unroll
         for (int i = 0; i < 2 * CT; ++i) gmax[i] = -CUDART_INF_F;
 
-        auto process = [&](uint32_t (&v)[32], int col0, int ci, bool odd) {
+        auto process = [&](uint32_t (&v)[32], int col0, int ci, bool odd, bool offd, float tau_c) {
             if (dbg & 1) { if (__uint_as_float(v[0] ^ v[31]) == 12345.678f) thr_cur = 0.f; return; }
             float m[11];
             auto tree = [&]() {
@@ -544,6 +590,42 @@
                     ++ev_n; ev_cyc += dt; ev_max = dt > ev_max ? dt : ev_max;
                 }
             }
+            if (!SEED && offd) {
+                const bool row_ok = thr_cur != CUDART_INF_F;
+                float tmin = fminf(tau_c, __shfl_down_sync(0xffffffffu, tau_c, 1));
+                tmin = fminf(tmin, __shfl_down_sync(0xffffffffu, tau_c, 2));
+                unsigned tm = 0u;
+#pragma unroll
+                for (int i = 0; i < 11; ++i) tm |= (m[i] > __shfl_sync(0xffffffffu, tmin, 3 * i) ? 1u : 0u) << i;
+                const unsigned tu = __reduce_or_sync(0xffffffffu, row_ok ? tm : 0u);
+                if (tu != 0u) {
+                    unsigned hm = 0u;
+#pragma unroll
+                    for (int i = 0; i < 11; ++i) {
+                        if ((tu >> i) & 1u) {
+#pragma unroll
+                            for (int e = 0; e < 3; ++e) {
+                                if (3 * i + e < 32) {
+                                    const float tk = __shfl_sync(0xffffffffu, tau_c, 3 * i + e);
+                                    hm |= (row_ok && ((tm >> i) & 1u) && __uint_as_float(v[3 * i + e]) > tk ? 1u : 0u) << (3 * i + e);
+                                }
+                            }
+                        }
+                    }
+                    while (hm) {
+                        const int k = __ffs(hm) - 1;
+                        hm &= hm - 1u;
+                        const unsigned at = atomicAdd(q_head, 1u);
+                        while ((int)(at - *q_tail) >= (int)qcap) __nanosleep(20);
+                        const unsigned e = at & (qcap - 1);
+                        q_ent[4 * e] = make_float4(select32(v, k), __int_as_float(grow), 0.f, 0.f);
+                        q_ent[4 * e + 2] = make_float4(0.f, 0.f, 0.f, __int_as_float(col0 + k));
+                        q_ent[4 * e + 3] = make_float4(__int_as_float(-1), 0.f, 0.f, 0.f);
+                        __threadfence_block();
+                        q_flag[e] = 1;
+                    }
+                }
+            }
         };
 
         uint32_t va[32], vb[32];
@@ -551,17 +633,22 @@
         uint32_t taddr_e = ((uint32_t)(quarter * 32) << 16) + (uint32_t)(SPLIT ? (slice & 1) * 128 + (slice >> 1) * 64 : slice * CPT);
         uint32_t bar_tf_e = bar_tfull + 8u * (SPLIT ? (uint32_t)(slice & 1) : 0u);
         uint32_t bar_te_e = mapa_cluster(bar_tempty, 0);
-        for (int tt = 0, t = t_start; tt < T; ++tt, t = (t + 1 == t_end) ? t_beg : t + 1) {
+        auto col_tau = [&](int c0) { return c0 + lane < n ? __ldcg(p.col_thr + c0 + lane) : CUDART_INF_F; };
+        const Sweep sw = sweep();
+        for (int tt = 0, t = t_start; tt < sw.len; ++tt, t = next_tile(t, sw)) {
             asm volatile("" : "+r"(taddr_e), "+r"(bar_tf_e), "+r"(bar_te_e));
             const uint32_t par = (uint32_t)tt & 1u;
             const uint32_t acc_phase = (uint32_t)(tt >> 1) & 1u;
+            const int col0 = t * BN + tile_col;
+            const bool offd = !SEED && p.sym && t != sw.last;
+            float tau0 = 0.f, tau1 = 0.f;
+            if (CPT == 64 && offd) { tau0 = col_tau(col0); tau1 = col_tau(col0 + 32); }
             mbar_wait(bar_tf_e + par * (SPLIT ? 16u : 8u), acc_phase);
             tc_fence_after();
             const bool tr = trc && blockIdx.x == 0 && blockIdx.y == 0 && tt < 64 && threadIdx.x == kNonEpiThreads;
             if (tr) trc[tt * 8 + 2] = clock64();
             if (!SEED) thr_cur = fmaxf(thr_cur, row_thr[r]);
             const uint32_t taddr = taddr_e + par * (uint32_t)(SPLIT ? 256 : BN);
-            const int col0 = t * BN + tile_col;
             const bool odd = (t & 1) != 0;
             if (CPT == 64) {
                 if (!(dbg & 2)) {
@@ -573,15 +660,17 @@
                 __syncwarp();
                 if (lane == 0) mbar_arrive_remote(bar_te_e + 8u * par);
                 if (tr) trc[tt * 8 + 3] = clock64();
-                process(va, col0, 0, odd);
-                process(vb, col0 + 32, CT > 1 ? 1 : 0, odd);
+                process(va, col0, 0, odd, offd, tau0);
+                process(vb, col0 + 32, CT > 1 ? 1 : 0, odd, offd, tau1);
             } else {
                 tmem_ld32(taddr, va);
 #pragma unroll
                 for (int c = 0; c < CT; c += 2) {
                     tmem_ld_wait();
                     tmem_ld32(taddr + (c + 1) * 32, vb);
-                    process(va, col0 + c * 32, c, odd);
+                    tau0 = offd ? col_tau(col0 + c * 32) : 0.f;
+                    tau1 = offd ? col_tau(col0 + (c + 1) * 32) : 0.f;
+                    process(va, col0 + c * 32, c, odd, offd, tau0);
                     tmem_ld_wait();
                     if (c + 2 < CT) tmem_ld32(taddr + (c + 2) * 32, va);
                     else {
@@ -589,7 +678,7 @@
                         __syncwarp();
                         if (lane == 0) mbar_arrive_remote(bar_te_e + 8u * par);
                     }
-                    process(vb, col0 + (c + 1) * 32, c + 1, odd);
+                    process(vb, col0 + (c + 1) * 32, c + 1, odd, offd, tau1);
                 }
             }
         }
@@ -613,7 +702,7 @@
     if (life) {
         unsigned long long ns1; asm volatile("mov.u64 %0, %%globaltimer;" : "=l"(ns1));
         long long* o = trc + 512 + (blockIdx.x == 0 ? 0 : 4);
-        o[0] = clock64() - life_clk; o[1] = (long long)(ns1 - life_ns); o[2] = T; o[3] = blockIdx.x;
+        o[0] = clock64() - life_clk; o[1] = (long long)(ns1 - life_ns); o[2] = sweep().len; o[3] = blockIdx.x;
     }
     cluster_sync_all();
     if (warp == 2) {
@@ -632,17 +721,26 @@
 }
 __device__ __forceinline__ bool better(float sa, int ia, float sb, int ib) { return sa > sb || (sa == sb && ia < ib); }
 
+__global__ void __launch_bounds__(256) simknn_col_thr_kernel(const float* __restrict__ seeds, int n, int remove_self, int seed_stride, int seed_q,
+                                                            float thr_lo, float* __restrict__ col_thr) {
+    for (int j = blockIdx.x * blockDim.x + threadIdx.x; j < n; j += gridDim.x * blockDim.x)
+        col_thr[j] = seed_threshold(seeds, j, j, remove_self, seed_stride, seed_q, thr_lo);
+}
+
 __global__ void __launch_bounds__(256) simknn_rescore_kernel(
     const float* __restrict__ xq, const float* __restrict__ xall, int64_t ld32, int d4, int nq, int n, int q_offset, int remove_self, int m_total,
     int nsplit, int top_k, float thr, float eps, const float* __restrict__ cand_val, const int* __restrict__ cand_idx,
     const float* __restrict__ cand_min,
     int* __restrict__ idx_out, float* __restrict__ sim_out, int* __restrict__ cnt_out, int* __restrict__ fb_rows, int* __restrict__ n_fallback,
-    const int* __restrict__ nq_dev, const int* __restrict__ row_map) {
+    const int* __restrict__ nq_dev, const int* __restrict__ row_map,
+    int col_cap, const int* __restrict__ col_cnt, const int* __restrict__ col_idx, const unsigned short* __restrict__ col_val,
+    const int* __restrict__ col_ovf) {
     extern __shared__ float sm2[];
     const int warp = threadIdx.x >> 5, lane = threadIdx.x & 31;
-    const int m3 = 3 * m_total;
-    float* sc = sm2 + (size_t)warp * 2 * m3;
-    int* id = reinterpret_cast<int*>(sc + m3);
+    const unsigned lt = (1u << lane) - 1u;
+    const int m3 = 3 * m_total, mw = m3 + col_cap;
+    float* sc = sm2 + (size_t)warp * 2 * mw;
+    int* id = reinterpret_cast<int*>(sc + mw);
     if (nq_dev) nq = min(nq, __ldg(nq_dev));
     for (int f = blockIdx.x * 8 + warp; f < nq; f += gridDim.x * 8) {
         const int row = row_map ? __ldg(row_map + f) : f;
@@ -664,49 +762,62 @@
                 continue;
             }
         }
-        for (int m = lane; m < m_total; m += 32)
-            sc[m] = __ldg(cand_idx + (size_t)f * m_total + m) >= 0 ? __ldg(cand_val + (size_t)f * m_total + m) : -CUDART_INF_F;
+        const int ccnt = col_cap > 0 ? min(__ldg(col_cnt + row), col_cap) : 0;
+        const int* cidx = col_idx + (size_t)row * col_cap;
+        const unsigned short* cval = col_val + (size_t)row * col_cap;
+        int nent = 0;
+        for (int m0 = 0; m0 < m_total + ccnt; m0 += 32) {
+            const int m = m0 + lane;
+            float v = 0.f; bool ok = false;
+            if (m < m_total) { ok = __ldg(cand_idx + (size_t)f * m_total + m) >= 0; v = __ldg(cand_val + (size_t)f * m_total + m); }
+            else if (m < m_total + ccnt) { ok = true; v = q_upper(__ldg(cval + m - m_total)); }
+            const unsigned b = __ballot_sync(0xffffffffu, ok);
+            if (ok) sc[nent + __popc(b & lt)] = v;
+            nent += __popc(b);
+        }
         __syncwarp();
-        float tk = CUDART_INF_F; int ntrip = 0;
-        for (int m0 = 0; m0 < m_total; m0 += 32) {
+        float tk = CUDART_INF_F;
+        for (int m0 = 0; m0 < nent; m0 += 32) {
             const int m = m0 + lane;
-            const float v = m < m_total ? sc[m] : -CUDART_INF_F;
-            int above = 0;
-            for (int o = 0; o < m_total; ++o) above += sc[o] > v ? 1 : 0;
-            if (v > -CUDART_INF_F && above < top_k) tk = fminf(tk, v);
-            ntrip += __popc(__ballot_sync(0xffffffffu, v > -CUDART_INF_F));
+            if (m < nent) {
+                const float v = sc[m];
+                int above = 0;
+                for (int o = 0; o < nent; ++o) above += sc[o] > v ? 1 : 0;
+                if (above < top_k) tk = fminf(tk, v);
+            }
         }
 #pragma unroll
         for (int o = 16; o > 0; o >>= 1) tk = fminf(tk, __shfl_xor_sync(0xffffffffu, tk, o));
-        const float cutoff = ntrip >= top_k ? tk - 2.0f * eps - 2.0f * kQBin : -CUDART_INF_F;
+        const float cutoff = nent >= top_k ? tk - 2.0f * eps - 2.0f * kQBin : -CUDART_INF_F;
         __syncwarp();
         int nvalid = 0;
-        for (int m0 = 0; m0 < m3; m0 += 32) {
+        for (int m0 = 0; m0 < m3 + ccnt; m0 += 32) {
             const int m = m0 + lane;
-            int j = -1; float s = -CUDART_INF_F;
+            int j = -1;
             if (m < m3) {
                 const int base = __ldg(cand_idx + (size_t)f * m_total + m / 3), e = m % 3;
                 if (base >= 0 && __ldg(cand_val + (size_t)f * m_total + m / 3) >= cutoff && (e < 2 || (base & 31) != 30) && base + e < n &&
-                    base + e != self_col) {
+                    base + e != self_col)
                     j = base + e;
-                    s = dot_seq(a, xall + (int64_t)j * ld32, d4);
-                }
-                sc[m] = s; id[m] = j;
-            }
-            nvalid += __popc(__ballot_sync(0xffffffffu, j >= 0 && s >= thr));
+            } else if (m < m3 + ccnt) {
+                if (q_upper(__ldg(cval + m - m3)) >= cutoff) j = __ldg(cidx + m - m3);
+            }
+            const float s = j >= 0 ? dot_seq(a, xall + (int64_t)j * ld32, d4) : -CUDART_INF_F;
+            const bool keep = j >= 0 && s >= thr;
+            const unsigned b = __ballot_sync(0xffffffffu, keep);
+            if (keep) { sc[nvalid + __popc(b & lt)] = s; id[nvalid + __popc(b & lt)] = j; }
+            nvalid += __popc(b);
         }
         __syncwarp();
         const int cnt = min(nvalid, top_k);
         float kth = thr;
-        for (int m0 = 0; m0 < m3; m0 += 32) {
+        for (int m0 = 0; m0 < nvalid; m0 += 32) {
             const int m = m0 + lane;
             int rank = 0x7fffffff; float s = 0.f; int j = -1;
-            if (m < m3) {
+            if (m < nvalid) {
                 s = sc[m]; j = id[m];
-                if (j >= 0 && s >= thr) {
-                    rank = 0;
-                    for (int o = 0; o < m3; ++o) rank += (id[o] >= 0 && better(sc[o], id[o], s, j)) ? 1 : 0;
-                }
+                rank = 0;
+                for (int o = 0; o < nvalid; ++o) rank += better(sc[o], id[o], s, j) ? 1 : 0;
             }
             if (rank < top_k) {
                 idx_out[(size_t)row * top_k + rank] = j;
@@ -718,6 +829,7 @@
         for (int t = cnt + lane; t < top_k; t += 32) { idx_out[(size_t)row * top_k + t] = -1; sim_out[(size_t)row * top_k + t] = 0.f; }
         float bound = -CUDART_INF_F;
         for (int s0 = lane; s0 < nsplit; s0 += 32) bound = fmaxf(bound, __ldg(cand_min + (size_t)f * nsplit + s0) + eps);
+        if (col_cap > 0 && lane == 0) bound = fmaxf(bound, fkey_inv(__ldg(col_ovf + row)) + eps);
 #pragma unroll
         for (int o = 16; o > 0; o >>= 1) bound = fmaxf(bound, __shfl_xor_sync(0xffffffffu, bound, o));
         if (lane == 0) {
@@ -1057,6 +1169,21 @@
     return SNG_OK;
 }
 
+struct ColLists {
+    int cap;
+    float* thr;
+    int *cnt, *ovf, *idx;
+    unsigned short* val;
+};
+
+static bool sym_eligible(const Plan& pl, int64_t nq, int64_t q_offset, int64_t n) {
+    return q_offset == 0 && nq == n && pl.nsplit == 1 && !env_flag("SNG_KNN_NOSYM");
+}
+static int col_cap_for(const Plan& pl) {
+    const int o = env_int("SNG_KNN_COLCAP", 1, kMaxCandTotal - pl.lists() * pl.cand);
+    return o ? o : kMaxCandTotal - pl.lists() * pl.cand;
+}
+
 template <int EW, bool SEED>
 static cudaError_t launch_ew(dim3 grid, size_t smem, cudaStream_t st, const CUtensorMap& mq, const CUtensorMap& mdb, const Stage1Params& p) {
     cudaError_t e = cudaFuncSetAttribute(simknn_stage1_kernel<EW, SEED>, cudaFuncAttributeMaxDynamicSharedMemorySize, (int)smem);
@@ -1067,7 +1194,8 @@
 
 static int launch_stage1(const Plan& pl, const uint16_t* xq, const uint16_t* xall, int64_t ldb, int64_t nq, int64_t q_offset, int64_t n,
                          float thr_lo, int remove_self, float* cand_val, int* cand_idx, float* cand_min, const float* seeds,
-                         float* seed_out, int* phase, cudaStream_t st, const int* nq_dev = nullptr, const int* row_ids = nullptr) {
+                         float* seed_out, int* phase, cudaStream_t st, const int* nq_dev = nullptr, const int* row_ids = nullptr,
+                         const ColLists* cl = nullptr) {
     const bool seed_pass = seed_out != nullptr;
     const int64_t n_db = seed_pass ? (n + pl.seed_stride - 1) / pl.seed_stride : n;
     CUtensorMap mq, mdb;
@@ -1084,6 +1212,9 @@
     p.phase = seed_pass ? nullptr : phase;
     p.nq_dev = nq_dev; p.row_ids = row_ids;
     p.seeds = seed_pass ? nullptr : seeds; p.seed_out = seed_out; p.seed_q = pl.seed_q; p.seed_stride = pl.seed_stride > 0 ? pl.seed_stride : 1;
+    p.sym = cl != nullptr;
+    p.col_cap = cl ? cl->cap : 0; p.col_thr = cl ? cl->thr : nullptr; p.col_cnt = cl ? cl->cnt : nullptr; p.col_ovf = cl ? cl->ovf : nullptr;
+    p.col_idx = cl ? cl->idx : nullptr; p.col_val = cl ? cl->val : nullptr;
     dim3 grid((unsigned)(2 * ((nq + 2 * BM - 1) / (2 * BM))), (unsigned)p.nsplit);
     p.trace = nullptr;
     if (env_flag("SNG_KNN_TRACE") && !seed_pass) {
@@ -1138,6 +1269,7 @@
 using namespace sng::knn;
 
 static size_t align256(size_t x) { return (x + 255) / 256 * 256; }
+static size_t col_bytes(int64_t n, int cap) { return 3 * align256((size_t)n * 4) + align256((size_t)n * cap * 4) + align256((size_t)n * cap * 2); }
 
 extern "C" int sng_set_debug_env(int enabled) { const int was = sng::knn::g_debug_env; sng::knn::g_debug_env = enabled ? 1 : 0; return was; }
 
@@ -1150,7 +1282,7 @@
     return align256(slots * 4) * 2 + align256((size_t)nq * pl.lists() * 4) + align256((size_t)nq * 4) + 2 * align256(part * 4) +
            align256((size_t)nq * kSeedGroups * 4) + 256 +
            align256((size_t)retry_rows(nq) * retry_ld(d) * 2) + 2 * align256((size_t)retry_rows(nq) * kMaxCandTotal * 4) + align256((size_t)retry_rows(nq) * 8 * 4) +
-           align256((size_t)nq * 4) + 256 + 1024;
+           align256((size_t)nq * 4) + 256 + 1024 + (sym_eligible(pl, nq, 0, n) ? col_bytes(n, col_cap_for(pl)) : 0);
 }
 
 extern "C" int sng_simknn_plan(int64_t nq, int64_t n, int64_t d, int top_k, int32_t* out8) {
@@ -1223,7 +1355,17 @@
     int* rcand_idx = reinterpret_cast<int*>(w); w += align256((size_t)kRetryRows * kMaxCandTotal * 4);
     float* rcand_min = reinterpret_cast<float*>(w); w += align256((size_t)kRetryRows * 8 * 4);
     int* fb2_rows = reinterpret_cast<int*>(w); w += align256((size_t)nq * 4);
-    int* n_fb1 = reinterpret_cast<int*>(w);
+    int* n_fb1 = reinterpret_cast<int*>(w); w += 256;
+    ColLists cl{};
+    const bool sym = sym_eligible(pl, nq, q_offset, n);
+    if (sym) {
+        cl.cap = col_cap_for(pl);
+        cl.thr = reinterpret_cast<float*>(w); w += align256((size_t)n * 4);
+        cl.cnt = reinterpret_cast<int*>(w); w += align256((size_t)n * 4);
+        cl.ovf = reinterpret_cast<int*>(w); w += align256((size_t)n * 4);
+        cl.idx = reinterpret_cast<int*>(w); w += align256((size_t)n * cl.cap * 4);
+        cl.val = reinterpret_cast<unsigned short*>(w);
+    }
     Plan pr;
     bool retry = false;
     if (!env_flag("SNG_KNN_NORETRY")) {
@@ -1246,19 +1388,29 @@
     if (cudaMemsetAsync(phase, 0, 8 * sizeof(int), st) != cudaSuccess) return check_launch("sng_simknn_build memset");
     if (cudaMemsetAsync(n_fb1, 0, sizeof(int), st) != cudaSuccess) return check_launch("sng_simknn_build memset");
     if (cudaMemsetAsync(n_fallback, 0, sizeof(int), st) != cudaSuccess) return check_launch("sng_simknn_build memset");
+    if (sym && (cudaMemsetAsync(cl.cnt, 0, (size_t)n * 4, st) != cudaSuccess ||
+                cudaMemsetAsync(cl.ovf, 0x80, (size_t)n * 4, st) != cudaSuccess))
+        return check_launch("sng_simknn_build memset");
     const float thr_lo = thr - 1.01f * eps;
     if (pl.seed_stride > 0)
         if (int rc = launch_stage1(pl, xq, xall, ldb, nq, q_offset, n, thr_lo, remove_self, nullptr, nullptr, nullptr, nullptr, seeds, nullptr, st)) return rc;
+    if (sym) {
+        const int blocks = (int)((n + 255) / 256 < (int64_t)sm_count() * 8 ? (n + 255) / 256 : (int64_t)sm_count() * 8);
+        simknn_col_thr_kernel<<<blocks > 0 ? blocks : 1, 256, 0, st>>>(pl.seed_stride > 0 ? seeds : nullptr, (int)n, remove_self,
+                                                                      pl.seed_stride > 0 ? pl.seed_stride : 1, pl.seed_q, thr_lo, cl.thr);
+        if (int rc = check_launch("simknn column thresholds")) return rc;
+    }
     if (int rc = launch_stage1(pl, xq, xall, ldb, nq, q_offset, n, thr_lo, remove_self, cand_val, cand_idx, cand_min,
-                               pl.seed_stride > 0 ? seeds : nullptr, nullptr, env_flag("SNG_KNN_NOPHASE") ? nullptr : phase, st)) return rc;
+                               pl.seed_stride > 0 ? seeds : nullptr, nullptr, env_flag("SNG_KNN_NOPHASE") ? nullptr : phase, st,
+                               nullptr, nullptr, sym ? &cl : nullptr)) return rc;
     const int d4 = (int)((d + 3) / 4);
     int* flag_rows = retry ? fb_rows : fb2_rows;
     int* flag_cnt = retry ? n_fb1 : n_fallback;
     {
         const int blocks = (int)((nq + 7) / 8 < (int64_t)sm_count() * 8 ? (nq + 7) / 8 : (int64_t)sm_count() * 8);
-        simknn_rescore_kernel<<<blocks > 0 ? blocks : 1, 256, (size_t)8 * 2 * 3 * m_total * 4, st>>>(
+        simknn_rescore_kernel<<<blocks > 0 ? blocks : 1, 256, (size_t)8 * 2 * (3 * m_total + cl.cap) * 4, st>>>(
             xq32, xall32, ld32, d4, (int)nq, (int)n, (int)q_offset, remove_self, m_total, pl.lists(), top_k, thr, eps, cand_val, cand_idx, cand_min,
-            idx, sim, cnt, flag_rows, flag_cnt, nullptr, nullptr);
+            idx, sim, cnt, flag_rows, flag_cnt, nullptr, nullptr, cl.cap, cl.cnt, cl.idx, cl.val, cl.ovf);
         if (int rc = check_launch("simknn stage 2")) return rc;
     }
     if (retry) {
@@ -1288,7 +1440,7 @@
             const int rblocks = (n_launch + 7) / 8 < 4096 ? (n_launch + 7) / 8 : 4096;
             simknn_rescore_kernel<<<rblocks, 256, (size_t)8 * 2 * 3 * mr * 4, st>>>(
                 xq32, xall32, ld32, d4, n_launch, (int)n, (int)q_offset, remove_self, mr, pr.lists(), top_k, thr, eps, rcand_val, rcand_idx, rcand_min,
-                idx, sim, cnt, fb2_rows, n_fallback, round_cnt + r, rows_r);
+                idx, sim, cnt, fb2_rows, n_fallback, round_cnt + r, rows_r, 0, nullptr, nullptr, nullptr, nullptr);
         }
         if (int rc = check_launch("simknn retry pass")) return rc;
     }
```

Result: faster. 7334, median of 6 (+7.5%).
